# valida-xyz/valida

Measured on AMD Instinct MI355X. Metric: proofs/sec, 2^20-row Fibonacci trace, higher is better.
Workload: dtype u32; 1 GPU; C2: Fibonacci 2^20 cpu rows (mem 2^22), 14 chips, one proof per GPU; field=BabyBear / Ext5, mmcs=Keccak-256, fri_blowup=2, log_blowup=1, num_queries=40, pow_bits=8, parallelism=single GPU, proofs_in_flight_per_gpu=3, comm_stuck=False

## Files before the change

### bindings/rust/src/lib.rs

```rust
#![allow(non_camel_case_types, dead_code)]
use core::ffi::{c_char, c_int, c_void};

pub const VGPU_CBOR_CANONICAL_FIELDS: u32 = 1;
pub const VGPU_CBOR_PLAIN_DIGESTS: u32 = 2;
pub const VGPU_CBOR_IN_BARE_IS_MONTGOMERY: u32 = 1;
pub const VGPU_CBOR_SAW_FIELD_STRUCT: u32 = 1;
pub const VGPU_CBOR_SAW_FIELD_BARE: u32 = 2;
pub const VGPU_CBOR_SAW_DIGEST_STRUCT: u32 = 4;
pub const VGPU_CBOR_SAW_DIGEST_PLAIN: u32 = 8;
pub const VGPU_COMM_ID_BYTES: u32 = 128;
pub const VGPU_OK: i32 = 0;
pub const VGPU_ERR_INVALID_ARG: i32 = -1;
pub const VGPU_ERR_OOM: i32 = -2;
pub const VGPU_ERR_HIP: i32 = -3;
pub const VGPU_ERR_UNSUPPORTED: i32 = -4;
pub const VGPU_ERR_INTERNAL: i32 = -5;
pub const VGPU_ERR_FABRIC: i32 = -6;
pub const VGPU_HASH_KECCAK256: i32 = 0;
pub const VGPU_HASH_POSEIDON16: i32 = 1;
pub const VGPU_CPU_STORE32: i32 = 0;
pub const VGPU_CPU_LOAD32: i32 = 1;
pub const VGPU_CPU_JAL: i32 = 2;
pub const VGPU_CPU_JALV: i32 = 3;
pub const VGPU_CPU_BEQ: i32 = 4;
// ... 276 lines not shown
    pub alu2: [*const VgpuAluOp; 4],
    pub n_alu2: [u64; 4],
    pub output: *const VgpuOutOp,
    pub n_output: u64,
}

#[link(name = "vgpu")]
extern "C" {
    pub fn vgpu_last_error() -> *const c_char;
    pub fn vgpu_version() -> *const c_char;
    pub fn vgpu_air_new(name: *const c_char, width: u32, preprocessed_width: u32, out: *mut *mut VgpuAir) -> i32;
    pub fn vgpu_air_free(air: *mut VgpuAir);
    pub fn vgpu_air_constant(air: *mut VgpuAir, canonical: u32) -> u32;
    pub fn vgpu_air_variable(air: *mut VgpuAir, is_preprocessed: u32, column: u32, is_next: u32) -> u32;
    pub fn vgpu_air_is_first_row(air: *mut VgpuAir) -> u32;
    pub fn vgpu_air_is_last_row(air: *mut VgpuAir) -> u32;
    pub fn vgpu_air_is_transition(air: *mut VgpuAir) -> u32;
    pub fn vgpu_air_add(air: *mut VgpuAir, a: u32, b: u32) -> u32;
    pub fn vgpu_air_sub(air: *mut VgpuAir, a: u32, b: u32) -> u32;
    pub fn vgpu_air_mul(air: *mut VgpuAir, a: u32, b: u32) -> u32;
    pub fn vgpu_air_neg(air: *mut VgpuAir, a: u32) -> u32;
    pub fn vgpu_air_assert_zero(air: *mut VgpuAir, node: u32);
    pub fn vgpu_air_add_interaction(air: *mut VgpuAir, it: *const VgpuInteraction) -> i32;
    pub fn vgpu_machine_new(out: *mut *mut VgpuMachine) -> i32;
    pub fn vgpu_machine_push_air(m: *mut VgpuMachine, air: *const VgpuAir) -> i32;
    pub fn vgpu_machine_basic(out: *mut *mut VgpuMachine) -> i32;
    pub fn vgpu_machine_basic_via_ffi(out: *mut *mut VgpuMachine) -> i32;
    pub fn vgpu_machine_free(m: *mut VgpuMachine);
    pub fn vgpu_machine_num_chips(m: *const VgpuMachine) -> u32;
    pub fn vgpu_machine_chip_info(m: *const VgpuMachine, chip: u32, out: *mut u32) -> i32;
    pub fn vgpu_machine_interaction_words(m: *const VgpuMachine, chip: u32, out: *mut u32, cap: u64) -> i64;
    pub fn vgpu_machine_eval_constraints(m: *const VgpuMachine, chip: u32, main_local: *const u32, main_next: *const u32, prep_local: *const u32, prep_next: *const u32, is_first: u32, is_last: u32, is_transition: u32, out: *mut u32, cap: u32) -> i32;
    pub fn vgpu_challenger_new(poseidon_rc: *const u32, out: *mut *mut VgpuChallenger) -> i32;
    pub fn vgpu_challenger_free(ch: *mut VgpuChallenger);
    pub fn vgpu_challenger_observe(ch: *mut VgpuChallenger, values: *const u32, n: u64);
    pub fn vgpu_challenger_sample(ch: *mut VgpuChallenger, out: *mut u32, n: u64);
    pub fn vgpu_challenger_sample_bits(ch: *mut VgpuChallenger, bits: u32) -> u64;
    pub fn vgpu_challenger_grind(ch: *mut VgpuChallenger, bits: u32) -> u32;
    pub fn vgpu_poseidon16_permute(poseidon_rc: *const u32, state: *mut u32);
    pub fn vgpu_poseidon16_permute_sparse(poseidon_rc: *const u32, state: *mut u32) -> i32;
    pub fn vgpu_prover_create(cfg: *const VgpuConfig, machine: *const VgpuMachine, out: *mut *mut VgpuProver) -> i32;
    pub fn vgpu_prover_destroy(p: *mut VgpuProver);
    pub fn vgpu_prover_memory(p: *const VgpuProver, live_bytes: *mut u64, peak_bytes: *mut u64);
    pub fn vgpu_prover_trim(p: *mut VgpuProver) -> u64;
    pub fn vgpu_prover_memory_reset_peak(p: *mut VgpuProver);
    pub fn vgpu_prover_set_dense_lane(p: *mut VgpuProver, on: u32, min_nodes: u64);
    pub fn vgpu_prover_set_const_columns(p: *mut VgpuProver, on: u32);
    pub fn vgpu_prover_lane_stats(p: *const VgpuProver, entered: *mut u64, waited: *mut u64);
    pub fn vgpu_prover_set_profiling(p: *mut VgpuProver, on: u32);
    pub fn vgpu_prover_set_prep_cache(p: *mut VgpuProver, on: u32);
    pub fn vgpu_prover_set_profiling_filter(p: *mut VgpuProver, kernel_name: *const c_char);
    pub fn vgpu_prover_profile(p: *mut VgpuProver, out: *mut c_char, cap: u64) -> i64;
    pub fn vgpu_shader_clock_probe(device: i32, iters: u32, out: *mut u64) -> i32;
    pub fn vgpu_host_alloc(bytes: u64, out: *mut *mut c_void) -> i32;
    pub fn vgpu_host_free(ptr: *mut c_void);
    pub fn vgpu_trace_upload(p: *mut VgpuProver, data: *const u32, height: u64, width: u64, out: *mut *mut VgpuTrace) -> i32;
    pub fn vgpu_trace_free(t: *mut VgpuTrace);
    pub fn vgpu_commit_batches(p: *mut VgpuProver, mats: *const *const VgpuTrace, n_mats: u32, coset_shifts: *const u32, root: *mut u32, out: *mut *mut VgpuPdata) -> i32;
    pub fn vgpu_commit_batches_flagged(p: *mut VgpuProver, mats: *const *const VgpuTrace, n_mats: u32, root: *mut u32, out: *mut *mut VgpuPdata, varies_out: *mut u32) -> i32;
    pub fn vgpu_pdata_lde(p: *mut VgpuProver, pd: *const VgpuPdata, idx: u32, out: *mut u32, cap_words: u64) -> i32;
    pub fn vgpu_pdata_num_matrices(pd: *const VgpuPdata) -> u32;
    pub fn vgpu_pdata_lde_view(pd: *const VgpuPdata, idx: u32, out: *mut VgpuLdeView) -> i32;
    pub fn vgpu_pdata_free(pd: *mut VgpuPdata);
    pub fn vgpu_perm_trace(p: *mut VgpuProver, chip: u32, main: *const VgpuTrace, preprocessed_or_null: *const VgpuTrace, challenges: *const u32, out: *mut u32, cap_words: u64, cumulative_sum: *mut u32) -> i32;
    pub fn vgpu_perm_trace_device(p: *mut VgpuProver, chip: u32, main: *const VgpuTrace, preprocessed_or_null: *const VgpuTrace, challenges: *const u32, out: *mut *mut VgpuTrace, cumulative_sum: *mut u32) -> i32;
    pub fn vgpu_quotient(p: *mut VgpuProver, chip: u32, prep_pd: *const VgpuPdata, prep_idx: u32, main_pd: *const VgpuPdata, main_idx: u32, perm_pd: *const VgpuPdata, perm_idx: u32, perm_challenges: *const u32, alpha: *const u32, cumulative_sum: *const u32, out: *mut *mut VgpuTrace) -> i32;
    pub fn vgpu_open_multi_batches(p: *mut VgpuProver, rounds: *const *const VgpuPdata, n_rounds: u32, n_points: *const u32, points: *const u32, ch: *mut VgpuChallenger, out: *mut *mut VgpuOpening) -> i32;
    pub fn vgpu_opening_values_len(o: *const VgpuOpening) -> u64;
    pub fn vgpu_opening_values(o: *const VgpuOpening) -> *const u32;
    pub fn vgpu_opening_proof_len(o: *const VgpuOpening) -> u64;
    pub fn vgpu_opening_proof(o: *const VgpuOpening) -> *const u32;
    pub fn vgpu_opening_free(o: *mut VgpuOpening);
    pub fn vgpu_verify_multi_batches(cfg: *const VgpuConfig, commits: *const u32, n_rounds: u32, n_mats: *const u32, heights: *const u64, widths: *const u32, n_points: *const u32, points: *const u32, values: *const u32, n_value_words: u64, proof: *const u32, n_proof_words: u64, ch: *mut VgpuChallenger) -> i32;
    pub fn vgpu_verify(cfg: *const VgpuConfig, machine: *const VgpuMachine, preprocessed_commit: *const u32, proof_words: *const u32, n_words: u64) -> i32;
    pub fn vgpu_verifier_create(cfg: *const VgpuConfig, machine: *const VgpuMachine, out: *mut *mut VgpuVerifier) -> i32;
    pub fn vgpu_verifier_destroy(v: *mut VgpuVerifier);
    pub fn vgpu_verifier_set_chunk_words(v: *mut VgpuVerifier, chunk_words: u64) -> i32;
    pub fn vgpu_verify_batch(v: *mut VgpuVerifier, proofs: *const *const u32, n_words: *const u64, preprocessed_commits: *const u32, n_proofs: u32, status: *mut i32) -> i32;
    pub fn vgpu_verifier_message(v: *const VgpuVerifier, i: u32, out: *mut c_char, cap: u64) -> i64;
    pub fn vgpu_verifier_timing(v: *const VgpuVerifier, host_ms: *mut f64, device_ms: *mut f64);
    pub fn vgpu_host_commit_root(cfg: *const VgpuConfig, mats: *const *const u32, heights: *const u64, widths: *const u64, n_mats: u32, coset_shifts: *const u32, root: *mut u32) -> i32;
    pub fn vgpu_fri_fold(p: *mut VgpuProver, f: *const u32, n: u64, beta: *const u32, out: *mut u32) -> i32;
    pub fn vgpu_field_probe(p: *mut VgpuProver, op: u32, operands: *const u32, operand_words: u64, n_items: u64, results: *mut u32, result_words: u64) -> i32;
    pub fn vgpu_prover_set_pool_poison(p: *mut VgpuProver, mode: u32, word: u32) -> i32;
    pub fn vgpu_prover_pool_poison_stats(p: *const VgpuProver, out: *mut u64);
    pub fn vgpu_prover_pool_peek(p: *mut VgpuProver, bytes: u64, out: *mut u32, n_words: u64) -> i32;
    pub fn vgpu_verifier_set_poison(v: *mut VgpuVerifier, on: u32, word: u32) -> i32;
    pub fn vgpu_prove(p: *mut VgpuProver, main: *const *const VgpuTrace, n_main: u32, prep_chips: *const u32, prep: *const *const VgpuTrace, n_prep: u32, debug_flags: u32, out: *mut *mut VgpuProof) -> i32;
    pub fn vgpu_prove_async(p: *mut VgpuProver, main: *const *const VgpuTrace, n_main: u32, prep_chips: *const u32, prep: *const *const VgpuTrace, n_prep: u32, out: *mut *mut VgpuTicket) -> i32;
    pub fn vgpu_ticket_wait(t: *mut VgpuTicket, out: *mut *mut VgpuProof) -> i32;
    pub fn vgpu_proof_cbor(proof_words: *const u32, n_words: u64, flags: u32, out: *mut u8, cap_bytes: u64) -> i64;
    pub fn vgpu_proof_from_cbor(bytes: *const u8, n_bytes: u64, out: *mut u32, cap_words: u64) -> i64;
    pub fn vgpu_proof_from_cbor_ex(bytes: *const u8, n_bytes: u64, flags: u32, out: *mut u32, cap_words: u64, forms_seen: *mut u32) -> i64;
    pub fn vgpu_proof_len(pr: *const VgpuProof) -> u64;
    pub fn vgpu_proof_words(pr: *const VgpuProof) -> *const u32;
    pub fn vgpu_proof_phase_ms(pr: *const VgpuProof, out: *mut f64);
    pub fn vgpu_proof_transcript(pr: *const VgpuProof, out: *mut u32);
    pub fn vgpu_proof_debug_perm_trace(pr: *const VgpuProof, chip: u32, out: *mut u32, cap_words: u64) -> i64;
    pub fn vgpu_proof_debug_quotient(pr: *const VgpuProof, chip: u32, out: *mut u32, cap_words: u64) -> i64;
    pub fn vgpu_proof_free(pr: *mut VgpuProof);
    pub fn vgpu_bus_audit(p: *mut VgpuProver, main: *const *const VgpuTrace, n_main: u32, prep_chips: *const u32, prep: *const *const VgpuTrace, n_prep: u32, opts: *const VgpuBusAuditOpts, out: *mut *mut VgpuBusReport) -> i32;
    pub fn vgpu_bus_audit_host(machine: *const VgpuMachine, main: *const *const u32, heights: *const u64, widths: *const u64, n_main: u32, prep_chips: *const u32, prep: *const *const u32, prep_heights: *const u64, prep_widths: *const u64, n_prep: u32, opts: *const VgpuBusAuditOpts, out: *mut *mut VgpuBusReport) -> i32;
    pub fn vgpu_bus_report_len(r: *const VgpuBusReport) -> u64;
    pub fn vgpu_bus_report_words(r: *const VgpuBusReport) -> *const u32;
    pub fn vgpu_bus_report_timing(r: *const VgpuBusReport, out: *mut f64);
    pub fn vgpu_bus_report_free(r: *mut VgpuBusReport);
    pub fn vgpu_constraint_audit(p: *mut VgpuProver, main: *const *const VgpuTrace, n_main: u32, prep_chips: *const u32, prep: *const *const VgpuTrace, n_prep: u32, opts: *const VgpuConstraintAuditOpts, out: *mut *mut VgpuConstraintReport) -> i32;
    pub fn vgpu_constraint_audit_host(machine: *const VgpuMachine, main: *const *const u32, heights: *const u64, widths: *const u64, n_main: u32, prep_chips: *const u32, prep: *const *const u32, prep_heights: *const u64, prep_widths: *const u64, n_prep: u32, opts: *const VgpuConstraintAuditOpts, out: *mut *mut VgpuConstraintReport) -> i32;
    pub fn vgpu_constraint_report_len(r: *const VgpuConstraintReport) -> u64;
    pub fn vgpu_constraint_report_words(r: *const VgpuConstraintReport) -> *const u32;
    pub fn vgpu_constraint_report_timing(r: *const VgpuConstraintReport, out: *mut f64);
    pub fn vgpu_constraint_report_free(r: *mut VgpuConstraintReport);
    pub fn vgpu_mutation_audit(p: *mut VgpuProver, main: *const *const VgpuTrace, n_main: u32, prep_chips: *const u32, prep: *const *const VgpuTrace, n_prep: u32, opts: *const VgpuMutationAuditOpts, out: *mut *mut VgpuMutationReport) -> i32;
    pub fn vgpu_mutation_audit_host(machine: *const VgpuMachine, main: *const *const u32, heights: *const u64, widths: *const u64, n_main: u32, prep_chips: *const u32, prep: *const *const u32, prep_heights: *const u64, prep_widths: *const u64, n_prep: u32, opts: *const VgpuMutationAuditOpts, out: *mut *mut VgpuMutationReport) -> i32;
    pub fn vgpu_mutation_report_len(r: *const VgpuMutationReport) -> u64;
    pub fn vgpu_mutation_report_words(r: *const VgpuMutationReport) -> *const u32;
    pub fn vgpu_mutation_report_timing(r: *const VgpuMutationReport, out: *mut f64);
    pub fn vgpu_mutation_report_free(r: *mut VgpuMutationReport);
    pub fn vgpu_pair_audit(p: *mut VgpuProver, main: *const *const VgpuTrace, n_main: u32, prep_chips: *const u32, prep: *const *const VgpuTrace, n_prep: u32, opts: *const VgpuPairAuditOpts, out: *mut *mut VgpuPairReport) -> i32;
    pub fn vgpu_pair_audit_host(machine: *const VgpuMachine, main: *const *const u32, heights: *const u64, widths: *const u64, n_main: u32, prep_chips: *const u32, prep: *const *const u32, prep_heights: *const u64, prep_widths: *const u64, n_prep: u32, opts: *const VgpuPairAuditOpts, out: *mut *mut VgpuPairReport) -> i32;
    pub fn vgpu_pair_report_len(r: *const VgpuPairReport) -> u64;
    pub fn vgpu_pair_report_words(r: *const VgpuPairReport) -> *const u32;
    pub fn vgpu_pair_report_timing(r: *const VgpuPairReport, out: *mut f64);
    pub fn vgpu_pair_report_free(r: *mut VgpuPairReport);
    pub fn vgpu_rank_audit(p: *mut VgpuProver, main: *const *const VgpuTrace, n_main: u32, prep_chips: *const u32, prep: *const *const VgpuTrace, n_prep: u32, opts: *const VgpuRankAuditOpts, out: *mut *mut VgpuRankReport) -> i32;
    pub fn vgpu_rank_audit_host(machine: *const VgpuMachine, main: *const *const u32, heights: *const u64, widths: *const u64, n_main: u32, prep_chips: *const u32, prep: *const *const u32, prep_heights: *const u64, prep_widths: *const u64, n_prep: u32, opts: *const VgpuRankAuditOpts, out: *mut *mut VgpuRankReport) -> i32;
    pub fn vgpu_rank_report_len(r: *const VgpuRankReport) -> u64;
    pub fn vgpu_rank_report_words(r: *const VgpuRankReport) -> *const u32;
    pub fn vgpu_rank_report_timing(r: *const VgpuRankReport, out: *mut f64);
    pub fn vgpu_rank_report_free(r: *mut VgpuRankReport);
    pub fn vgpu_field_audit(p: *mut VgpuProver, main: *const *const VgpuTrace, n_main: u32, prep_chips: *const u32, prep: *const *const VgpuTrace, n_prep: u32, opts: *const VgpuRankAuditOpts, out: *mut *mut VgpuFieldReport) -> i32;
    pub fn vgpu_field_audit_host(machine: *const VgpuMachine, main: *const *const u32, heights: *const u64, widths: *const u64, n_main: u32, prep_chips: *const u32, prep: *const *const u32, prep_heights: *const u64, prep_widths: *const u64, n_prep: u32, opts: *const VgpuRankAuditOpts, out: *mut *mut VgpuFieldReport) -> i32;
    pub fn vgpu_field_report_len(r: *const VgpuFieldReport) -> u64;
    pub fn vgpu_field_report_words(r: *const VgpuFieldReport) -> *const u32;
    pub fn vgpu_field_report_timing(r: *const VgpuFieldReport, out: *mut f64);
    pub fn vgpu_field_report_free(r: *mut VgpuFieldReport);
    pub fn vgpu_link_audit(p: *mut VgpuProver, main: *const *const VgpuTrace, n_main: u32, prep_chips: *const u32, prep: *const *const VgpuTrace, n_prep: u32, opts: *const VgpuLinkAuditOpts, out: *mut *mut VgpuLinkReport) -> i32;
    pub fn vgpu_link_audit_host(machine: *const VgpuMachine, main: *const *const u32, heights: *const u64, widths: *const u64, n_main: u32, prep_chips: *const u32, prep: *const *const u32, prep_heights: *const u64, prep_widths: *const u64, n_prep: u32, opts: *const VgpuLinkAuditOpts, out: *mut *mut VgpuLinkReport) -> i32;
    pub fn vgpu_link_report_len(r: *const VgpuLinkReport) -> u64;
    pub fn vgpu_link_report_words(r: *const VgpuLinkReport) -> *const u32;
    pub fn vgpu_link_report_timing(r: *const VgpuLinkReport, out: *mut f64);
    pub fn vgpu_link_report_free(r: *mut VgpuLinkReport);
    pub fn vgpu_step_audit(p: *mut VgpuProver, main: *const *const VgpuTrace, n_main: u32, prep_chips: *const u32, prep: *const *const VgpuTrace, n_prep: u32, opts: *const VgpuStepAuditOpts, out: *mut *mut VgpuStepReport) -> i32;
    pub fn vgpu_step_audit_host(machine: *const VgpuMachine, main: *const *const u32, heights: *const u64, widths: *const u64, n_main: u32, prep_chips: *const u32, prep: *const *const u32, prep_heights: *const u64, prep_widths: *const u64, n_prep: u32, opts: *const VgpuStepAuditOpts, out: *mut *mut VgpuStepReport) -> i32;
    pub fn vgpu_step_report_len(r: *const VgpuStepReport) -> u64;
    pub fn vgpu_step_report_words(r: *const VgpuStepReport) -> *const u32;
    pub fn vgpu_step_report_timing(r: *const VgpuStepReport, out: *mut f64);
    pub fn vgpu_step_report_free(r: *mut VgpuStepReport);
    pub fn vgpu_invariant_audit(p: *mut VgpuProver, main: *const *const VgpuTrace, n_main: u32, prep_chips: *const u32, prep: *const *const VgpuTrace, n_prep: u32, opts: *const VgpuInvariantAuditOpts, out: *mut *mut VgpuInvariantReport) -> i32;
    pub fn vgpu_invariant_audit_host(machine: *const VgpuMachine, main: *const *const u32, heights: *const u64, widths: *const u64, n_main: u32, prep_chips: *const u32, prep: *const *const u32, prep_heights: *const u64, prep_widths: *const u64, n_prep: u32, opts: *const VgpuInvariantAuditOpts, out: *mut *mut VgpuInvariantReport) -> i32;
    pub fn vgpu_invariant_report_len(r: *const VgpuInvariantReport) -> u64;
    pub fn vgpu_invariant_report_words(r: *const VgpuInvariantReport) -> *const u32;
    pub fn vgpu_invariant_report_timing(r: *const VgpuInvariantReport, out: *mut f64);
    pub fn vgpu_invariant_report_free(r: *mut VgpuInvariantReport);
    pub fn vgpu_transition_audit(p: *mut VgpuProver, main: *const *const VgpuTrace, n_main: u32, prep_chips: *const u32, prep: *const *const VgpuTrace, n_prep: u32, opts: *const VgpuTransitionAuditOpts, out: *mut *mut VgpuTransitionReport) -> i32;
    pub fn vgpu_transition_audit_host(machine: *const VgpuMachine, main: *const *const u32, heights: *const u64, widths: *const u64, n_main: u32, prep_chips: *const u32, prep: *const *const u32, prep_heights: *const u64, prep_widths: *const u64, n_prep: u32, opts: *const VgpuTransitionAuditOpts, out: *mut *mut VgpuTransitionReport) -> i32;
    pub fn vgpu_transition_report_len(r: *const VgpuTransitionReport) -> u64;
    pub fn vgpu_transition_report_words(r: *const VgpuTransitionReport) -> *const u32;
    pub fn vgpu_transition_report_timing(r: *const VgpuTransitionReport, out: *mut f64);
    pub fn vgpu_transition_report_free(r: *mut VgpuTransitionReport);
    pub fn vgpu_product_audit(p: *mut VgpuProver, main: *const *const VgpuTrace, n_main: u32, prep_chips: *const u32, prep: *const *const VgpuTrace, n_prep: u32, opts: *const VgpuProductAuditOpts, out: *mut *mut VgpuProductReport) -> i32;
    pub fn vgpu_product_audit_host(machine: *const VgpuMachine, main: *const *const u32, heights: *const u64, widths: *const u64, n_main: u32, prep_chips: *const u32, prep: *const *const u32, prep_heights: *const u64, prep_widths: *const u64, n_prep: u32, opts: *const VgpuProductAuditOpts, out: *mut *mut VgpuProductReport) -> i32;
    pub fn vgpu_product_report_len(r: *const VgpuProductReport) -> u64;
    pub fn vgpu_product_report_words(r: *const VgpuProductReport) -> *const u32;
    pub fn vgpu_product_report_timing(r: *const VgpuProductReport, out: *mut f64);
    pub fn vgpu_product_report_free(r: *mut VgpuProductReport);
// ... 58 lines not shown
```

### include/vgpu.h

```cpp
#ifndef VGPU_H
#define VGPU_H
#include <stdint.h>
#ifdef __cplusplus
extern "C" {
#endif

enum {
    VGPU_OK = 0,
    VGPU_ERR_INVALID_ARG = -1,
    VGPU_ERR_OOM = -2,
    VGPU_ERR_HIP = -3,
    VGPU_ERR_UNSUPPORTED = -4,
    VGPU_ERR_INTERNAL = -5,
    VGPU_ERR_FABRIC = -6
};
enum {
    VGPU_HASH_KECCAK256 = 0,
    VGPU_HASH_POSEIDON16 = 1
};

const char* vgpu_last_error(void);
const char* vgpu_version(void);

typedef struct vgpu_config {
// ... 54 lines not shown
uint32_t vgpu_challenger_grind(vgpu_challenger_t* ch, uint32_t bits);
void vgpu_poseidon16_permute(const uint32_t poseidon_rc[480], uint32_t state[16]);
int32_t vgpu_poseidon16_permute_sparse(const uint32_t poseidon_rc[480], uint32_t state[16]);

typedef struct vgpu_prover vgpu_prover_t;
typedef struct vgpu_trace vgpu_trace_t;
typedef struct vgpu_pdata vgpu_pdata_t;
typedef struct vgpu_proof vgpu_proof_t;

int32_t vgpu_prover_create(const vgpu_config_t* cfg, const vgpu_machine_t* machine, vgpu_prover_t** out);
void vgpu_prover_destroy(vgpu_prover_t* p);
void vgpu_prover_memory(const vgpu_prover_t* p, uint64_t* live_bytes, uint64_t* peak_bytes);
uint64_t vgpu_prover_trim(vgpu_prover_t* p);
void vgpu_prover_memory_reset_peak(vgpu_prover_t* p);
void vgpu_prover_set_dense_lane(vgpu_prover_t* p, uint32_t on, uint64_t min_nodes);
void vgpu_prover_set_const_columns(vgpu_prover_t* p, uint32_t on);
void vgpu_prover_lane_stats(const vgpu_prover_t* p, uint64_t* entered, uint64_t* waited);

void vgpu_prover_set_profiling(vgpu_prover_t* p, uint32_t on);
void vgpu_prover_set_prep_cache(vgpu_prover_t* p, uint32_t on);
void vgpu_prover_set_profiling_filter(vgpu_prover_t* p, const char* kernel_name);
int64_t vgpu_prover_profile(vgpu_prover_t* p, char* out, uint64_t cap);
int32_t vgpu_shader_clock_probe(int32_t device, uint32_t iters, uint64_t out[2]);

int32_t vgpu_host_alloc(uint64_t bytes, void** out);
void vgpu_host_free(void* ptr);

int32_t vgpu_trace_upload(vgpu_prover_t* p, const uint32_t* data, uint64_t height, uint64_t width, vgpu_trace_t** out);
void vgpu_trace_free(vgpu_trace_t* t);

int32_t vgpu_commit_batches(vgpu_prover_t* p, const vgpu_trace_t* const* mats, uint32_t n_mats, const uint32_t* coset_shifts,
                            uint32_t root[8], vgpu_pdata_t** out);
int32_t vgpu_commit_batches_flagged(vgpu_prover_t* p, const vgpu_trace_t* const* mats, uint32_t n_mats, uint32_t root[8], vgpu_pdata_t** out,
                                    uint32_t* varies_out);
int32_t vgpu_pdata_lde(vgpu_prover_t* p, const vgpu_pdata_t* pd, uint32_t idx, uint32_t* out, uint64_t cap_words);
typedef struct vgpu_lde_view {
    const uint32_t* data;
    uint64_t height, width, stride;
    uint32_t log_blowup;
} vgpu_lde_view_t;
uint32_t vgpu_pdata_num_matrices(const vgpu_pdata_t* pd);
int32_t vgpu_pdata_lde_view(const vgpu_pdata_t* pd, uint32_t idx, vgpu_lde_view_t* out);
void vgpu_pdata_free(vgpu_pdata_t* pd);

int32_t vgpu_perm_trace(vgpu_prover_t* p, uint32_t chip, const vgpu_trace_t* main, const vgpu_trace_t* preprocessed_or_null,
                        const uint32_t challenges[15], uint32_t* out, uint64_t cap_words, uint32_t cumulative_sum[5]);

int32_t vgpu_perm_trace_device(vgpu_prover_t* p, uint32_t chip, const vgpu_trace_t* main, const vgpu_trace_t* preprocessed_or_null,
                               const uint32_t challenges[15], vgpu_trace_t** out, uint32_t cumulative_sum[5]);

int32_t vgpu_quotient(vgpu_prover_t* p, uint32_t chip, const vgpu_pdata_t* prep_pd, uint32_t prep_idx, const vgpu_pdata_t* main_pd, uint32_t main_idx,
                      const vgpu_pdata_t* perm_pd, uint32_t perm_idx, const uint32_t perm_challenges[15], const uint32_t alpha[5],
                      const uint32_t cumulative_sum[5], vgpu_trace_t** out);

typedef struct vgpu_opening vgpu_opening_t;
int32_t vgpu_open_multi_batches(vgpu_prover_t* p, const vgpu_pdata_t* const* rounds, uint32_t n_rounds, const uint32_t* n_points,
                                const uint32_t* points, vgpu_challenger_t* ch, vgpu_opening_t** out);
uint64_t vgpu_opening_values_len(const vgpu_opening_t* o);
const uint32_t* vgpu_opening_values(const vgpu_opening_t* o);
uint64_t vgpu_opening_proof_len(const vgpu_opening_t* o);
const uint32_t* vgpu_opening_proof(const vgpu_opening_t* o);
void vgpu_opening_free(vgpu_opening_t* o);

int32_t vgpu_verify_multi_batches(const vgpu_config_t* cfg, const uint32_t* commits, uint32_t n_rounds, const uint32_t* n_mats, const uint64_t* heights,
                                  const uint32_t* widths, const uint32_t* n_points, const uint32_t* points, const uint32_t* values, uint64_t n_value_words,
                                  const uint32_t* proof, uint64_t n_proof_words, vgpu_challenger_t* ch);

int32_t vgpu_verify(const vgpu_config_t* cfg, const vgpu_machine_t* machine, const uint32_t* preprocessed_commit, const uint32_t* proof_words,
                    uint64_t n_words);
typedef struct vgpu_verifier vgpu_verifier_t;
int32_t vgpu_verifier_create(const vgpu_config_t* cfg, const vgpu_machine_t* machine, vgpu_verifier_t** out);
void vgpu_verifier_destroy(vgpu_verifier_t* v);
int32_t vgpu_verifier_set_chunk_words(vgpu_verifier_t* v, uint64_t chunk_words);
int32_t vgpu_verify_batch(vgpu_verifier_t* v, const uint32_t* const* proofs, const uint64_t* n_words, const uint32_t* preprocessed_commits,
                          uint32_t n_proofs, int32_t* status);
int64_t vgpu_verifier_message(const vgpu_verifier_t* v, uint32_t i, char* out, uint64_t cap);
void vgpu_verifier_timing(const vgpu_verifier_t* v, double* host_ms, double* device_ms);
int32_t vgpu_host_commit_root(const vgpu_config_t* cfg, const uint32_t* const* mats, const uint64_t* heights, const uint64_t* widths, uint32_t n_mats,
                              const uint32_t* coset_shifts, uint32_t root[8]);

int32_t vgpu_fri_fold(vgpu_prover_t* p, const uint32_t* f, uint64_t n, const uint32_t beta[5], uint32_t* out);

int32_t vgpu_field_probe(vgpu_prover_t* p, uint32_t op, const uint32_t* operands, uint64_t operand_words, uint64_t n_items, uint32_t* results, uint64_t result_words);

int32_t vgpu_prover_set_pool_poison(vgpu_prover_t* p, uint32_t mode, uint32_t word);
void vgpu_prover_pool_poison_stats(const vgpu_prover_t* p, uint64_t out[4]);
int32_t vgpu_prover_pool_peek(vgpu_prover_t* p, uint64_t bytes, uint32_t* out, uint64_t n_words);
int32_t vgpu_verifier_set_poison(vgpu_verifier_t* v, uint32_t on, uint32_t word);

int32_t vgpu_prove(vgpu_prover_t* p, const vgpu_trace_t* const* main, uint32_t n_main, const uint32_t* prep_chips,
                   const vgpu_trace_t* const* prep, uint32_t n_prep, uint32_t debug_flags, vgpu_proof_t** out);
typedef struct vgpu_ticket vgpu_ticket_t;
int32_t vgpu_prove_async(vgpu_prover_t* p, const vgpu_trace_t* const* main, uint32_t n_main, const uint32_t* prep_chips,
                         const vgpu_trace_t* const* prep, uint32_t n_prep, vgpu_ticket_t** out);
int32_t vgpu_ticket_wait(vgpu_ticket_t* t, vgpu_proof_t** out);
#define VGPU_CBOR_CANONICAL_FIELDS 1u
#define VGPU_CBOR_PLAIN_DIGESTS 2u
int64_t vgpu_proof_cbor(const uint32_t* proof_words, uint64_t n_words, uint32_t flags, uint8_t* out, uint64_t cap_bytes);
int64_t vgpu_proof_from_cbor(const uint8_t* bytes, uint64_t n_bytes, uint32_t* out, uint64_t cap_words);
#define VGPU_CBOR_IN_BARE_IS_MONTGOMERY 1u
#define VGPU_CBOR_SAW_FIELD_STRUCT 1u
#define VGPU_CBOR_SAW_FIELD_BARE 2u
#define VGPU_CBOR_SAW_DIGEST_STRUCT 4u
#define VGPU_CBOR_SAW_DIGEST_PLAIN 8u
int64_t vgpu_proof_from_cbor_ex(const uint8_t* bytes, uint64_t n_bytes, uint32_t flags, uint32_t* out, uint64_t cap_words, uint32_t* forms_seen);
uint64_t vgpu_proof_len(const vgpu_proof_t* pr);
const uint32_t* vgpu_proof_words(const vgpu_proof_t* pr);
void vgpu_proof_phase_ms(const vgpu_proof_t* pr, double out[11]);
void vgpu_proof_transcript(const vgpu_proof_t* pr, uint32_t out[33]);
int64_t vgpu_proof_debug_perm_trace(const vgpu_proof_t* pr, uint32_t chip, uint32_t* out, uint64_t cap_words);
int64_t vgpu_proof_debug_quotient(const vgpu_proof_t* pr, uint32_t chip, uint32_t* out, uint64_t cap_words);
void vgpu_proof_free(vgpu_proof_t* pr);

typedef struct vgpu_bus_audit_opts { uint64_t max_tuples; uint32_t max_records_per_tuple; uint32_t hash_bits; } vgpu_bus_audit_opts_t;
typedef struct vgpu_bus_report vgpu_bus_report_t;
int32_t vgpu_bus_audit(vgpu_prover_t* p, const vgpu_trace_t* const* main, uint32_t n_main, const uint32_t* prep_chips, const vgpu_trace_t* const* prep,
                       uint32_t n_prep, const vgpu_bus_audit_opts_t* opts, vgpu_bus_report_t** out);
int32_t vgpu_bus_audit_host(const vgpu_machine_t* machine, const uint32_t* const* main, const uint64_t* heights, const uint64_t* widths, uint32_t n_main,
                            const uint32_t* prep_chips, const uint32_t* const* prep, const uint64_t* prep_heights, const uint64_t* prep_widths, uint32_t n_prep,
                            const vgpu_bus_audit_opts_t* opts, vgpu_bus_report_t** out);
uint64_t vgpu_bus_report_len(const vgpu_bus_report_t* r);
const uint32_t* vgpu_bus_report_words(const vgpu_bus_report_t* r);
void vgpu_bus_report_timing(const vgpu_bus_report_t* r, double out[2]);
void vgpu_bus_report_free(vgpu_bus_report_t* r);

typedef struct vgpu_constraint_audit_opts { uint64_t max_constraints; uint32_t max_rows_per_constraint; uint32_t reserved; } vgpu_constraint_audit_opts_t;
typedef struct vgpu_constraint_report vgpu_constraint_report_t;
int32_t vgpu_constraint_audit(vgpu_prover_t* p, const vgpu_trace_t* const* main, uint32_t n_main, const uint32_t* prep_chips, const vgpu_trace_t* const* prep,
                              uint32_t n_prep, const vgpu_constraint_audit_opts_t* opts, vgpu_constraint_report_t** out);
int32_t vgpu_constraint_audit_host(const vgpu_machine_t* machine, const uint32_t* const* main, const uint64_t* heights, const uint64_t* widths, uint32_t n_main,
                                   const uint32_t* prep_chips, const uint32_t* const* prep, const uint64_t* prep_heights, const uint64_t* prep_widths, uint32_t n_prep,
                                   const vgpu_constraint_audit_opts_t* opts, vgpu_constraint_report_t** out);
uint64_t vgpu_constraint_report_len(const vgpu_constraint_report_t* r);
const uint32_t* vgpu_constraint_report_words(const vgpu_constraint_report_t* r);
void vgpu_constraint_report_timing(const vgpu_constraint_report_t* r, double out[2]);
void vgpu_constraint_report_free(vgpu_constraint_report_t* r);

typedef struct vgpu_mutation_audit_opts {
    uint64_t max_entries;
    uint32_t max_rows_per_entry;
    uint32_t n_deltas;
    uint32_t deltas[4];
    uint32_t reserved[2];
} vgpu_mutation_audit_opts_t;
typedef struct vgpu_mutation_report vgpu_mutation_report_t;
int32_t vgpu_mutation_audit(vgpu_prover_t* p, const vgpu_trace_t* const* main, uint32_t n_main, const uint32_t* prep_chips, const vgpu_trace_t* const* prep,
                            uint32_t n_prep, const vgpu_mutation_audit_opts_t* opts, vgpu_mutation_report_t** out);
int32_t vgpu_mutation_audit_host(const vgpu_machine_t* machine, const uint32_t* const* main, const uint64_t* heights, const uint64_t* widths, uint32_t n_main,
                                 const uint32_t* prep_chips, const uint32_t* const* prep, const uint64_t* prep_heights, const uint64_t* prep_widths, uint32_t n_prep,
                                 const vgpu_mutation_audit_opts_t* opts, vgpu_mutation_report_t** out);
uint64_t vgpu_mutation_report_len(const vgpu_mutation_report_t* r);
const uint32_t* vgpu_mutation_report_words(const vgpu_mutation_report_t* r);
void vgpu_mutation_report_timing(const vgpu_mutation_report_t* r, double out[3]);
void vgpu_mutation_report_free(vgpu_mutation_report_t* r);

typedef struct vgpu_pair_audit_opts {
    uint64_t max_entries;
    uint32_t max_rows_per_entry;
    uint32_t n_deltas;
    uint32_t deltas[4];
    uint32_t chip_mask;
    uint32_t reserved;
} vgpu_pair_audit_opts_t;
typedef struct vgpu_pair_report vgpu_pair_report_t;
int32_t vgpu_pair_audit(vgpu_prover_t* p, const vgpu_trace_t* const* main, uint32_t n_main, const uint32_t* prep_chips, const vgpu_trace_t* const* prep,
                        uint32_t n_prep, const vgpu_pair_audit_opts_t* opts, vgpu_pair_report_t** out);
// ... 290 lines not shown
```

### valida_amd/__init__.py

```python
import ctypes
import os

import numpy as np

P = 2013265921
NUM_CHIPS = 14
CHIP_NAMES = ["cpu", "program", "mem", "add", "sub", "mul", "div", "shift", "lt", "com", "bitwise", "output", "range", "static_data"]

_HERE = os.path.dirname(os.path.abspath(__file__))
_LIB_PATH = os.environ.get("VGPU_LIB_PATH") or os.path.join(_HERE, "libvgpu.so")

c_u32p = ctypes.POINTER(ctypes.c_uint32)
c_u64p = ctypes.POINTER(ctypes.c_uint64)


HASH_KECCAK256, HASH_POSEIDON16 = 0, 1


class VgpuError(RuntimeError):
    def __init__(self, code, msg):
        super().__init__("vgpu error %d: %s" % (code, msg))
        self.code = code


# ... 241 lines not shown
        w = np.zeros(int(n), dtype=np.uint32)
        L.vgpu_machine_interaction_words(self._h, ctypes.c_uint32(chip), w.ctypes.data_as(c_u32p), ctypes.c_uint64(w.size))
        return decode_interaction_words(w)

    def eval_constraints(self, chip, main_local, main_next, prep_local=None, prep_next=None, is_first=0, is_last=0, is_transition=1):
        info = self.chip_info(chip)
        pl = np.zeros(max(1, info["preprocessed_width"]), dtype=np.uint32) if prep_local is None else prep_local
        pn = np.zeros(max(1, info["preprocessed_width"]), dtype=np.uint32) if prep_next is None else prep_next
        a, ap = _u32(main_local)
        b, bp = _u32(main_next)
        c, cp = _u32(pl)
        d, dp = _u32(pn)
        out = np.zeros(max(1, info["constraints"]), dtype=np.uint32)
        n = lib().vgpu_machine_eval_constraints(self._h, ctypes.c_uint32(chip), ap, bp, cp, dp, ctypes.c_uint32(is_first), ctypes.c_uint32(is_last),
                                                ctypes.c_uint32(is_transition), out.ctypes.data_as(c_u32p), ctypes.c_uint32(out.size))
        if n < 0:
            _check(n)
        return out[:n]

    def __del__(self):
        if getattr(self, "_h", None):
            try:
                lib().vgpu_machine_free(self._h)
            except TypeError:
                pass
            self._h = None


class Challenger:

    def __init__(self, rc):
        self._rc, rcp = _u32(rc)
        self._h = ctypes.c_void_p()
        _check(lib().vgpu_challenger_new(rcp, ctypes.byref(self._h)))

    def observe(self, values):
        v, vp = _u32(values)
        lib().vgpu_challenger_observe(self._h, vp, ctypes.c_uint64(v.size))

    def sample(self, n=1):
        out = np.zeros(n, dtype=np.uint32)
        lib().vgpu_challenger_sample(self._h, out.ctypes.data_as(c_u32p), ctypes.c_uint64(n))
        return out

    def sample_bits(self, bits):
        return int(lib().vgpu_challenger_sample_bits(self._h, ctypes.c_uint32(bits)))

    def grind(self, bits):
        return int(lib().vgpu_challenger_grind(self._h, ctypes.c_uint32(bits)))

    def __del__(self):
        if getattr(self, "_h", None):
            try:
                lib().vgpu_challenger_free(self._h)
            except TypeError:
                pass
            self._h = None


def poseidon16_permute(rc, state):
    r, rp = _u32(rc)
    s = np.array(state, dtype=np.uint32)
    lib().vgpu_poseidon16_permute(rp, s.ctypes.data_as(c_u32p))
    return s


FIELD_PROBE_OPS = {name: (code, iw, ow) for code, (name, iw, ow) in enumerate([
    ("reduce_once", 1, 1), ("sub_mod", 2, 1), ("add", 2, 1), ("sub", 2, 1), ("neg", 1, 1), ("mul", 2, 1), ("monty_reduce", 2, 1), ("monty_reduce_wide", 2, 1),
    ("from_canonical", 1, 1), ("canonical", 1, 1), ("inv", 1, 1), ("ext_mul", 10, 5), ("ext_square", 5, 5), ("ext_scale", 6, 5), ("ext_inv", 5, 5),
    ("bfly_dit_lb0", 18, 16), ("bfly_dit", 18, 16), ("bfly_dif_lb0", 18, 16), ("bfly_dif", 18, 16), ("monty_signed", 2, 1), ("sbox", 1, 1), ("sbox_plus", 2, 1),
    ("permute", 16, 16), ("permute_plain", 16, 16)])}


def field_probe(prover, op, operands):
    code, iw, ow = FIELD_PROBE_OPS[op]
    a = np.ascontiguousarray(operands, dtype=np.uint32)
    if a.ndim != 2 or a.shape[1] != iw or a.shape[0] == 0:
        raise ValueError("field_probe(%s): operands must be a non-empty (n_items, %d) array" % (op, iw))
    n = a.shape[0]
    src = np.ascontiguousarray(a.T)
    out = np.zeros((ow, n), dtype=np.uint32)
    _check(lib().vgpu_field_probe(prover._h, ctypes.c_uint32(code), src.ctypes.data_as(c_u32p), ctypes.c_uint64(src.size), ctypes.c_uint64(n),
                                  out.ctypes.data_as(c_u32p), ctypes.c_uint64(out.size)))
    return np.ascontiguousarray(out.T)


class _PinnedBlock:
    def __init__(self, nbytes):
        self.ptr = ctypes.c_void_p()
        _check(lib().vgpu_host_alloc(ctypes.c_uint64(max(1, nbytes)), ctypes.byref(self.ptr)))

    def __del__(self):
        if getattr(self, "ptr", None):
            try:
                lib().vgpu_host_free(self.ptr)
            except TypeError:
                pass
            self.ptr = None


def pinned_empty(shape, dtype=np.uint32):
    shape = (shape,) if isinstance(shape, int) else tuple(shape)
    dt = np.dtype(dtype)
    n = int(np.prod(shape)) if shape else 1
    blk = _PinnedBlock(n * dt.itemsize)
    buf = (ctypes.c_char * max(1, n * dt.itemsize)).from_address(blk.ptr.value)
    buf._vgpu_block = blk
    return np.frombuffer(buf, dtype=dt, count=n).reshape(shape)


def pinned_copy(a):
    out = pinned_empty(a.shape, a.dtype)
    out[...] = a
    return out


class DeviceOplog:
    def __init__(self, prover, handle, nbytes):
        self._prover, self._h, self.nbytes = prover, handle, nbytes

    def __del__(self):
        if getattr(self, "_h", None):
            try:
                lib().vgpu_oplog_free(self._h)
            except TypeError:
                pass
            self._h = None


class DeviceTrace:
    def __init__(self, prover, handle, shape):
        self._prover, self._h, self.shape = prover, handle, shape

    def download(self):
        out = np.zeros(self.shape, dtype=np.uint32)
        _check(lib().vgpu_trace_download(self._prover._h, self._h, out.ctypes.data_as(c_u32p), ctypes.c_uint64(out.size)))
        return out

    def __del__(self):
        if getattr(self, "_h", None):
            try:
                lib().vgpu_trace_free(self._h)
            except TypeError:
                pass
            self._h = None


class ProverData:

    def __init__(self, prover, handle, root, shapes):
        self._prover, self._h, self.root, self._shapes = prover, handle, root, shapes

    def lde(self, idx):
        h, w = self._shapes[idx]
        H = h << self._prover.log_blowup
        out = np.zeros((H, w), dtype=np.uint32)
        _check(lib().vgpu_pdata_lde(self._prover._h, self._h, ctypes.c_uint32(idx), out.ctypes.data_as(c_u32p), ctypes.c_uint64(out.size)))
        return out

    def lde_view(self, idx):

        class _View(ctypes.Structure):
            _fields_ = [("data", ctypes.c_void_p), ("height", ctypes.c_uint64), ("width", ctypes.c_uint64), ("stride", ctypes.c_uint64), ("log_blowup", ctypes.c_uint32)]

        v = _View()
        _check(lib().vgpu_pdata_lde_view(self._h, ctypes.c_uint32(idx), ctypes.byref(v)))
# ... 1908 lines not shown
```

### valida_amd/build.py

```python
import concurrent.futures
import os
import subprocess
import sys

ROOT = os.path.dirname(os.path.dirname(os.path.abspath(__file__)))
CSRC = os.path.join(ROOT, "valida_amd", "csrc")
BUILD = os.path.join(ROOT, "build")
LIB = os.path.join(ROOT, "valida_amd", "libvgpu.so")

SOURCES = [
    "kernels/ntt.hip",
    "kernels/layout.hip",
    "kernels/merkle.hip",
    "kernels/poseidon_mmcs.hip",
    "kernels/perm.hip",
    "kernels/quotient.hip",
    "kernels/open.hip",
    "kernels/tracegen.hip",
    "kernels/verify.hip",
    "kernels/bus_audit.hip",
    "kernels/constraint_audit.hip",
    "kernels/mutation_audit.hip",
    "kernels/coverage_audit.hip",
    "kernels/pair_audit.hip",
    "kernels/rank_audit.hip",
    "kernels/field_audit.hip",
    "kernels/link_audit.hip",
    "kernels/step_audit.hip",
    "kernels/invariant_audit.hip",
    "kernels/transition_audit.hip",
    "kernels/product_audit.hip",
    "kernels/domain_audit.hip",
    "kernels/memory_audit.hip",
    "kernels/program_audit.hip",
    "kernels/field_probe.hip",
    "host/prover.cpp",
    "host/prover_audits.cpp",
    "host/sharded_prover.cpp",
    "capi.cpp",
]
FLAGS = ["--offload-arch=gfx950", "-O3", "-std=c++17", "-fPIC", "-Wno-unused-result"]


def _newer_than(target, deps):
    if not os.path.exists(target):
        return False
    t = os.path.getmtime(target)
    return all(os.path.getmtime(d) <= t for d in deps)


def _all_headers():
    out = []
    for base, _, files in os.walk(CSRC):
        for f in files:
            if f.endswith((".hpp", ".h", ".inc")):
                out.append(os.path.join(base, f))
    out.append(os.path.join(ROOT, "include", "vgpu.h"))
    return out


LAST = {"compiled": [], "reused": [], "linked": False}
_FORCE = False


def _compile(src):
    obj = os.path.join(BUILD, src.replace("/", "_") + ".o")
    path = os.path.join(CSRC, src)
    if not _FORCE and _newer_than(obj, [path] + _all_headers()):
        LAST["reused"].append(src)
        return obj
    LAST["compiled"].append(src)
    cmd = ["hipcc"] + FLAGS + ["-x", "hip", "-c", path, "-o", obj]
    r = subprocess.run(cmd, capture_output=True, text=True)
    if r.returncode != 0:
        raise RuntimeError("hipcc failed for %s:\n%s" % (src, r.stderr))
    return obj


def build_vgpu(force=False):
    global _FORCE
    os.makedirs(BUILD, exist_ok=True)
    LAST["compiled"], LAST["reused"], LAST["linked"] = [], [], False
    srcs = [os.path.join(CSRC, s) for s in SOURCES]
    if not force and _newer_than(LIB, srcs + _all_headers()):
        LAST["reused"] = list(SOURCES)
        return LIB
    _FORCE = bool(force)
    with concurrent.futures.ThreadPoolExecutor(max_workers=8) as ex:
        objs = list(ex.map(_compile, SOURCES))
    tmp = os.path.join(BUILD, "libvgpu.%d.so" % os.getpid())
    cmd = ["hipcc", "--offload-arch=gfx950", "-shared", "-fPIC", "-o", tmp] + objs + ["-ldl"]
    r = subprocess.run(cmd, capture_output=True, text=True)
    if r.returncode != 0:
        if os.path.exists(tmp):
            os.unlink(tmp)
        raise RuntimeError("link failed:\n" + r.stderr)
    os.replace(tmp, LIB)
    LAST["linked"] = True
    return LIB


if __name__ == "__main__":
    print(build_vgpu("--force" in sys.argv))
```

### valida_amd/csrc/capi.cpp

```cpp
#include "../../include/vgpu.h"
#include <algorithm>
#include <cstring>
#include <future>
#include <map>
#include <mutex>
#include <memory>
#include <string>
#include "host/cbor.hpp"
#include "host/comm.hpp"
#include "host/sharded.hpp"
#include "host/sharded_prover.hpp"
#include "host/verifier.hpp"
#include "host/machine_verifier.hpp"
#include "host/verify_batch.hpp"
#include "host/poseidon_opt.hpp"
#include "host/prover.hpp"
#include "workload/basic_vm.hpp"
#include "workload/executable.hpp"

using namespace vhost;

static thread_local std::string g_err;
static int32_t fail(int32_t code, const std::string& msg) { g_err = msg; return code; }
#define VG_TRY(...)                                                         \
// ... 805 lines not shown
        std::vector<HostMatrixView> v;
        for (uint32_t i = 0; i < n_mats; i++) { if (!mats[i]) throw std::invalid_argument("null matrix"); v.push_back({mats[i], heights[i], widths[i]}); }
        Digest8 d = host_commit_root(v, coset_shifts, cfg->log_blowup, mmcs);
        memcpy(root, d.data(), 32);
    })
}
uint64_t vgpu_opening_values_len(const vgpu_opening_t* o) { return o->values.size(); }
const uint32_t* vgpu_opening_values(const vgpu_opening_t* o) { return o->values.data(); }
uint64_t vgpu_opening_proof_len(const vgpu_opening_t* o) { return o->proof.size(); }
const uint32_t* vgpu_opening_proof(const vgpu_opening_t* o) { return o->proof.data(); }
void vgpu_opening_free(vgpu_opening_t* o) { delete o; }

int32_t vgpu_perm_trace(vgpu_prover_t* p, uint32_t chip, const vgpu_trace_t* main, const vgpu_trace_t* prep, const uint32_t challenges[15], uint32_t* out,
                        uint64_t cap_words, uint32_t cumulative_sum[5]) {
    VG_TRY({
        if (!p || !main || !challenges || !out) throw std::invalid_argument("null argument");
        const MachineDesc& md = p->p->machine();
        if (chip >= md.airs.size()) throw std::invalid_argument("bad chip index");
        const AirDesc& air = md.airs[chip];
        if (main->t->width != air.width) throw std::invalid_argument("trace width mismatch");
        DeviceCtx& c = p->p->ctx();
        c.activate();
        DMat m = ingest(c, *main->t);
        DMat pm;
        if (prep) pm = ingest(c, *prep->t);
        Ext5 rnd[3];
        for (int i = 0; i < 3; i++) for (int k = 0; k < 5; k++) rnd[i].c[k] = Fp::from_canonical(challenges[5 * i + k]);
        uint32_t M = (uint32_t)air.interactions.size();
        std::vector<uint32_t> pool;
        size_t maxf = 0;
        for (auto& it : air.interactions) { put_ext(pool, (it.is_local() ? rnd[0] : rnd[1]).pow((uint64_t)it.bus_index + 1)); maxf = std::max(maxf, it.fields.size()); }
        Ext5 bp = Ext5::one();
        for (size_t j = 0; j < maxf; j++) { put_ext(pool, bp); bp *= rnd[2]; }
        pool.push_back(0);
        DBuf pool_dev(&c, pool), iw(&c, air.interaction_words), scratch(&c, (size_t)vk::perm_scratch_words(m.height));
        DMat perm(&c, m.height, 5 * (M + 1));
        if (cap_words < perm.height * perm.width) throw std::invalid_argument("output buffer too small");
        vk::launch_perm_trace(c.stream, m.view(), prep ? pm.view() : vk::DMatView{nullptr, 0, 0, 0}, iw.data, pool_dev.data, M, perm.view(), scratch.data);
        DBuf tmp(&c, (size_t)(perm.height * perm.width));
        vk::launch_export_rows(c.stream, perm.view(), 0, perm.height, tmp.data);
        c.check_launch("perm trace");
        c.download(out, tmp.data, perm.height * perm.width * 4);
        if (cumulative_sum) for (int k = 0; k < 5; k++) cumulative_sum[k] = out[(perm.height - 1) * perm.width + 5 * M + k];
    })
}

int32_t vgpu_fri_fold(vgpu_prover_t* p, const uint32_t* f, uint64_t n, const uint32_t beta[5], uint32_t* out) {
    VG_TRY({
        if (!p || !f || !beta || !out || n < 4 || (n & (n - 1))) throw std::invalid_argument("fri_fold: n must be a power of two >= 4");
        DeviceCtx& c = p->p->ctx();
        c.activate();
        uint64_t half = n / 2, q = half / 2;
        std::vector<uint32_t> in(5 * n);
        std::vector<uint32_t> bw(5);
        for (uint64_t i = 0; i < n; i++) for (int k = 0; k < 5; k++) in[((i & 1) * 5 + k) * half + (i >> 1)] = Fp::from_canonical(f[5 * i + k]).v;
        for (int k = 0; k < 5; k++) bw[k] = Fp::from_canonical(beta[k]).v;
        DBuf din(&c, in), dbeta(&c, bw), dout(&c, (size_t)(5 * half));
        vk::launch_fri_fold(c.stream, din.data, n, dbeta.data, nullptr, c.tables, dout.data);
        c.check_launch("fri fold");
        std::vector<uint32_t> o(5 * half);
        c.download(o.data(), dout.data, o.size() * 4);
        for (uint64_t i = 0; i < half; i++) for (int k = 0; k < 5; k++) out[5 * i + k] = Fp::raw(o[((i & 1) * 5 + k) * q + (i >> 1)]).canonical();
    })
}

int32_t vgpu_field_probe(vgpu_prover_t* p, uint32_t op, const uint32_t* operands, uint64_t operand_words, uint64_t n_items, uint32_t* results, uint64_t result_words) {
    VG_TRY({
        int iw = 0, ow = 0;
        if (!p || !operands || !results) throw std::invalid_argument("null argument");
        if (!vk::field_probe_shape(op, &iw, &ow)) throw std::invalid_argument("field probe: unknown op");
        if (n_items == 0 || n_items > (1ull << 24)) throw std::invalid_argument("field probe: 1 .. 2^24 items");
        if (operand_words != n_items * (uint64_t)iw || result_words != n_items * (uint64_t)ow) throw std::invalid_argument("field probe: buffer sizes do not match the op's shape");
        vk::field_probe_check_twiddle_range(op, operands, n_items);
        DeviceCtx& c = p->p->ctx();
        c.activate();
        DBuf din(&c, (size_t)operand_words), dout(&c, (size_t)result_words);
        c.upload(din.data, operands, operand_words * 4);
        vk::launch_field_probe(c.stream, op, din.data, n_items, c.tables, c.poseidon_tab, c.poseidon_sparse, dout.data);
        c.check_launch("field probe");
        c.download(results, dout.data, result_words * 4);
    })
}

int32_t vgpu_prover_set_pool_poison(vgpu_prover_t* p, uint32_t mode, uint32_t word) {
    VG_TRY({
        if (!p) throw std::invalid_argument("null argument");
        if (mode > 3) throw std::invalid_argument("pool poison: mode is bit 0 (on alloc) | bit 1 (on release)");
        DeviceCtx& c = p->p->ctx();
        std::unique_lock<std::mutex> owner(c.prove_mu, std::try_to_lock);
        if (!owner.owns_lock() || c.async_pending.load() > 0) throw std::invalid_argument("pool poison: a proof or an audit is running on this context");
        std::lock_guard<std::mutex> lk(c.pool_mu);
        c.poison_mode = mode;
        c.poison_word = word;
    })
}
void vgpu_prover_pool_poison_stats(const vgpu_prover_t* p, uint64_t out[4]) {
    if (!p || !out) return;
    DeviceCtx& c = const_cast<vgpu_prover_t*>(p)->p->ctx();
    std::lock_guard<std::mutex> lk(c.pool_mu);
    for (int i = 0; i < 4; i++) out[i] = c.poison_stats[i];
}
int32_t vgpu_prover_pool_peek(vgpu_prover_t* p, uint64_t bytes, uint32_t* out, uint64_t n_words) {
    VG_TRY({
        if (!p || !out) throw std::invalid_argument("null argument");
        if (!bytes || n_words > bytes / 4) throw std::invalid_argument("pool peek: bytes >= 1 and 4 * n_words <= bytes");
        DeviceCtx& c = p->p->ctx();
        c.activate();
        const size_t rounded = ((size_t)bytes + 255) & ~(size_t)255;
        DBuf b(&c, (size_t)((bytes + 3) / 4));
        std::vector<uint32_t> w(n_words + 1);
        if (n_words) c.download(w.data(), b.data, n_words * 4);
        c.download(w.data() + n_words, b.data + rounded / 4 - 1, 4);
        memcpy(out, w.data(), w.size() * 4);
    })
}

static void check_trace(const vgpu_prover_t* p, const vgpu_trace_t* t, std::vector<std::shared_ptr<Prover>>* foreign = nullptr) {
    if (!t || !t->t) throw std::invalid_argument("null trace");
    if (t->owner == p->p) return;
    if (!foreign || t->owner->ctx().device != p->p->ctx().device) throw std::invalid_argument("trace belongs to another prover context");
    if (std::find(foreign->begin(), foreign->end(), t->owner) == foreign->end()) foreign->push_back(t->owner);
}
static void drain(const std::vector<std::shared_ptr<Prover>>& ctxs) {
    for (auto& q : ctxs) { q->ctx().activate(); q->ctx().sync(); }
}

int32_t vgpu_prove(vgpu_prover_t* p, const vgpu_trace_t* const* main, uint32_t n_main, const uint32_t* prep_chips, const vgpu_trace_t* const* prep,
                   uint32_t n_prep, uint32_t debug_flags, vgpu_proof_t** out) {
    VG_TRY({
        if (!p || !main || !out || (n_prep && (!prep || !prep_chips))) throw std::invalid_argument("null argument");
        std::vector<const DeviceTrace*> m;
        std::vector<std::shared_ptr<Prover>> foreign;
        for (uint32_t i = 0; i < n_main; i++) { check_trace(p, main[i], &foreign); m.push_back(main[i]->t.get()); }
        std::vector<std::pair<int, const DeviceTrace*>> pr;
        for (uint32_t i = 0; i < n_prep; i++) { check_trace(p, prep[i], &foreign); pr.push_back({(int)prep_chips[i], prep[i]->t.get()}); }
        drain(foreign);
        auto proof = std::make_unique<vgpu_proof>();
        proof->dbg.keep_matrices = (debug_flags & 1) != 0;
        proof->dbg.check_constraints = (debug_flags & 2) != 0;
        proof->words = p->p->prove(m, pr, &proof->tm, &proof->dbg);
        *out = proof.release();
    })
}

extern "C++" {
template <class Report> static auto report_evaluations(const Report& rep, int) -> decltype(rep.evaluations) { return rep.evaluations; }
template <class Report> static double report_evaluations(const Report&, long) { return 0; }
template <class Handle, class Report>
static Handle* audit_report_handle(const Report& rep) {
    auto h = std::make_unique<Handle>();
    h->words = rep.words(); h->device_ms = rep.device_ms; h->host_ms = rep.host_ms; h->evaluations = report_evaluations(rep, 0);
    return h.release();
}
template <class Handle, class Audit>
static int32_t audit_on_device(vgpu_prover_t* p, const vgpu_trace_t* const* main, uint32_t n_main, const uint32_t* prep_chips, const vgpu_trace_t* const* prep, uint32_t n_prep, Handle** out,
                        Audit&& audit) {
    VG_TRY({
        if (!p || !out || (n_main && !main) || (n_prep && (!prep || !prep_chips))) throw std::invalid_argument("null argument");
        std::vector<const DeviceTrace*> m;
        std::vector<std::shared_ptr<Prover>> foreign;
        for (uint32_t i = 0; i < n_main; i++) { check_trace(p, main[i], &foreign); m.push_back(main[i]->t.get()); }
        std::vector<std::pair<int, const DeviceTrace*>> pr;
        for (uint32_t i = 0; i < n_prep; i++) { check_trace(p, prep[i], &foreign); pr.push_back({(int)prep_chips[i], prep[i]->t.get()}); }
        drain(foreign);
        *out = audit_report_handle<Handle>(audit(m, pr));
    })
// ... 861 lines not shown
```

### valida_amd/csrc/field.hpp

```cpp
#pragma once
#include <cstdint>

#if defined(__HIPCC__)
#include <hip/hip_runtime.h>
#define VG_HD __host__ __device__ __forceinline__
#else
#define VG_HD inline
#endif

namespace vg {

constexpr uint32_t P = 0x78000001u;
constexpr uint32_t P_INV_NEG = 0x77ffffffu;
constexpr uint32_t R_MOD_P = 268435454u;
constexpr uint32_t R2_MOD_P = 1172168163u;
constexpr uint32_t GENERATOR = 31;
constexpr uint32_t TWO_ADIC_ROOT_27 = 0x1a427a41u;

#ifndef VG_MULHI_NOP
#define VG_MULHI_NOP 0
#endif
VG_HD uint32_t mul_lo_pinv(uint32_t lo) {
#if defined(__HIP_DEVICE_COMPILE__) && VG_MULHI_NOP == 2
    uint32_t o;
    asm("v_mul_lo_u32 %0, %1, %2\n\ts_nop 0" : "=v"(o) : "v"(lo), "v"(0x88000001u));
    return o;
#else
    return lo * 0x88000001u;
#endif
}
VG_HD uint32_t mul_hi_u32(uint32_t a, uint32_t b) {
#if defined(__HIP_DEVICE_COMPILE__) && VG_MULHI_NOP
    uint32_t o;
    asm("v_mul_hi_u32 %0, %1, %2\n\ts_nop 0" : "=v"(o) : "v"(a), "v"(b));
    return o;
#elif defined(__HIP_DEVICE_COMPILE__)
    return __umulhi(a, b);
#else
    return (uint32_t)(((uint64_t)a * b) >> 32);
#endif
}

#ifndef VG_CARRY_REDUCE
#define VG_CARRY_REDUCE 1
#endif
#if defined(__HIP_DEVICE_COMPILE__) && VG_CARRY_REDUCE == 2
VG_HD uint32_t reduce_once(uint32_t s) {
    uint32_t t, r;
    asm("v_subrev_co_u32_e32 %0, vcc, %3, %2\n\tv_cndmask_b32_e32 %1, %0, %2, vcc" : "=&v"(t), "=v"(r) : "v"(s), "v"(P) : "vcc");
    return r;
}
VG_HD uint32_t sub_mod(uint32_t a, uint32_t b) {
    uint32_t d, t, r;
    asm("v_sub_co_u32_e32 %0, vcc, %3, %4\n\tv_add_u32_e32 %1, %5, %0\n\tv_cndmask_b32_e32 %2, %0, %1, vcc" : "=&v"(d), "=&v"(t), "=v"(r) : "v"(a), "v"(b), "v"(P) : "vcc");
    return r;
}
#elif defined(__HIP_DEVICE_COMPILE__) && VG_CARRY_REDUCE
VG_HD uint32_t reduce_once(uint32_t s) {
    uint32_t t, r;
    unsigned long long borrow;
    asm("v_subrev_co_u32_e64 %0, %1, %4, %3\n\tv_cndmask_b32_e64 %2, %0, %3, %1" : "=&v"(t), "=&s"(borrow), "=v"(r) : "v"(s), "v"(P));
    return r;
}
VG_HD uint32_t sub_mod(uint32_t a, uint32_t b) {
    uint32_t d, t, r;
    unsigned long long borrow;
    asm("v_sub_co_u32_e64 %0, %1, %4, %5\n\tv_add_u32_e32 %2, %6, %0\n\tv_cndmask_b32_e64 %3, %0, %2, %1" : "=&v"(d), "=&s"(borrow), "=&v"(t), "=v"(r) : "v"(a), "v"(b), "v"(P));
    return r;
}
#else
VG_HD uint32_t reduce_once(uint32_t s) { uint32_t t = s - P; return s < t ? s : t; }
VG_HD uint32_t sub_mod(uint32_t a, uint32_t b) { uint32_t d = a - b, t = d + P; return d < t ? d : t; }
#endif

#ifndef VG_MONTY_ADD
#define VG_MONTY_ADD 0
#endif
VG_HD uint32_t monty_reduce(uint64_t t) {
#if VG_MONTY_ADD == 1
    const uint32_t m = (uint32_t)t * P_INV_NEG;
    return reduce_once((uint32_t)((t + (uint64_t)m * P) >> 32));
#else
    uint32_t lo = (uint32_t)t, hi = (uint32_t)(t >> 32);
    uint32_t m = mul_lo_pinv(lo);
    uint32_t u = mul_hi_u32(m, P);
    return sub_mod(hi, u);
#endif
}

VG_HD uint32_t monty_reduce_wide(uint64_t t) {
    uint32_t lo = (uint32_t)t, hi = reduce_once((uint32_t)(t >> 32));
    uint32_t m = mul_lo_pinv(lo);
    uint32_t u = mul_hi_u32(m, P);
    return sub_mod(hi, u);
}

struct Fp {
    uint32_t v;
    VG_HD static Fp raw(uint32_t m) { Fp r; r.v = m; return r; }
    VG_HD static Fp zero() { return raw(0); }
    VG_HD static Fp one() { return raw(R_MOD_P); }
    VG_HD static Fp from_canonical(uint32_t x) { return raw(monty_reduce((uint64_t)x * R2_MOD_P)); }
    VG_HD uint32_t canonical() const { return monty_reduce((uint64_t)v); }
    VG_HD bool is_zero() const { return v == 0; }
    VG_HD bool operator==(const Fp& o) const { return v == o.v; }
    VG_HD bool operator!=(const Fp& o) const { return v != o.v; }
    VG_HD Fp operator+(const Fp& o) const { return raw(reduce_once(v + o.v)); }
    VG_HD Fp operator-(const Fp& o) const { return raw(sub_mod(v, o.v)); }
    VG_HD Fp operator-() const { return raw(v ? P - v : 0); }
#if VG_MONTY_ADD == 2 && defined(__HIP_DEVICE_COMPILE__)
    VG_HD Fp operator*(const Fp& o) const {
        uint32_t lo, hi;
        asm("v_mul_lo_u32 %0, %2, %3\n\tv_mul_hi_u32 %1, %2, %3" : "=&v"(lo), "=v"(hi) : "v"(v), "v"(o.v));
        return raw(sub_mod(hi, mul_hi_u32(lo * 0x88000001u, P)));
    }
#else
    VG_HD Fp operator*(const Fp& o) const { return raw(monty_reduce((uint64_t)v * o.v)); }
#endif
    VG_HD Fp& operator+=(const Fp& o) { *this = *this + o; return *this; }
    VG_HD Fp& operator-=(const Fp& o) { *this = *this - o; return *this; }
    VG_HD Fp& operator*=(const Fp& o) { *this = *this * o; return *this; }
    VG_HD Fp square() const { return *this * *this; }
    VG_HD Fp pow(uint64_t e) const {
        Fp r = one(), b = *this;
        while (e) { if (e & 1) r *= b; b *= b; e >>= 1; }
        return r;
    }
    VG_HD Fp exp_power_of_2(unsigned k) const { Fp r = *this; for (unsigned i = 0; i < k; i++) r *= r; return r; }
    VG_HD Fp inv() const {
        const Fp x = *this;
        const Fp x3 = x.square() * x, x7 = x3.square() * x;
        const Fp a6 = x7.exp_power_of_2(3) * x7;
        const Fp a12 = a6.exp_power_of_2(6) * a6;
        const Fp a24 = a12.exp_power_of_2(12) * a12;
        const Fp t = a24.exp_power_of_2(3) * x7;
        const Fp w = t * x, w2 = w.square(), w4 = w2.square(), w8 = w4.square();
        return t * (w8 * w4 * w2);
    }
    VG_HD Fp halve() const { return raw((v & 1) ? (uint32_t)(((uint64_t)v + P) >> 1) : v >> 1); }
};

VG_HD Fp two_adic_generator(unsigned bits) {
    return Fp::from_canonical(TWO_ADIC_ROOT_27).exp_power_of_2(27 - bits);
}

struct Ext5 {
    Fp c[5];
    VG_HD static Ext5 zero() { Ext5 r; for (int i = 0; i < 5; i++) r.c[i] = Fp::zero(); return r; }
    VG_HD static Ext5 one() { Ext5 r = zero(); r.c[0] = Fp::one(); return r; }
    VG_HD static Ext5 from_base(Fp b) { Ext5 r = zero(); r.c[0] = b; return r; }
    VG_HD bool is_zero() const { return (c[0].v | c[1].v | c[2].v | c[3].v | c[4].v) == 0; }
    VG_HD bool operator==(const Ext5& o) const { for (int i = 0; i < 5; i++) if (c[i].v != o.c[i].v) return false; return true; }
    VG_HD bool operator!=(const Ext5& o) const { return !(*this == o); }
    VG_HD Ext5 operator+(const Ext5& o) const { Ext5 r; for (int i = 0; i < 5; i++) r.c[i] = c[i] + o.c[i]; return r; }
    VG_HD Ext5 operator-(const Ext5& o) const { Ext5 r; for (int i = 0; i < 5; i++) r.c[i] = c[i] - o.c[i]; return r; }
    VG_HD Ext5 operator-() const { Ext5 r; for (int i = 0; i < 5; i++) r.c[i] = -c[i]; return r; }
    VG_HD Ext5 operator*(const Fp& s) const { Ext5 r; for (int i = 0; i < 5; i++) r.c[i] = c[i] * s; return r; }
    VG_HD Ext5 operator+(const Fp& s) const { Ext5 r = *this; r.c[0] += s; return r; }
    VG_HD Ext5 operator-(const Fp& s) const { Ext5 r = *this; r.c[0] -= s; return r; }
    VG_HD Ext5 operator*(const Ext5& o) const {
        Fp d[5];
#pragma unroll
        for (int j = 0; j < 5; j++) d[j] = o.c[j] + o.c[j];
        Ext5 r;
#pragma unroll
        for (int k = 0; k < 5; k++) {
            uint32_t bb[5];
#pragma unroll
            for (int i = 0; i < 5; i++) bb[i] = i <= k ? o.c[k - i].v : d[k + 5 - i].v;
            uint64_t t0123 = (uint64_t)c[0].v * bb[0] + (uint64_t)c[1].v * bb[1] + (uint64_t)c[2].v * bb[2] + (uint64_t)c[3].v * bb[3];
            uint64_t t4 = (uint64_t)c[4].v * bb[4];
            r.c[k] = Fp::raw(monty_reduce_wide(t0123)) + Fp::raw(monty_reduce(t4));
        }
        return r;
    }
    VG_HD Ext5& operator+=(const Ext5& o) { *this = *this + o; return *this; }
    VG_HD Ext5& operator-=(const Ext5& o) { *this = *this - o; return *this; }
    VG_HD Ext5& operator*=(const Ext5& o) { *this = *this * o; return *this; }
    VG_HD Ext5 square() const { return *this * *this; }
    VG_HD Ext5 pow(uint64_t e) const {
        Ext5 r = one(), b = *this;
        while (e) { if (e & 1) r *= b; b *= b; e >>= 1; }
        return r;
    }
    VG_HD Ext5 exp_power_of_2(unsigned k) const { Ext5 r = *this; for (unsigned i = 0; i < k; i++) r *= r; return r; }
    template <int K> VG_HD Ext5 frobenius_k() const {
        constexpr uint32_t Z[5] = {0, 1079828539u, 847078768u, 1597816133u, 233372948u};
        Ext5 r;
        r.c[0] = c[0];
        r.c[1] = c[1] * Fp::raw(Z[(1 * K) % 5]);
        r.c[2] = c[2] * Fp::raw(Z[(2 * K) % 5]);
        r.c[3] = c[3] * Fp::raw(Z[(3 * K) % 5]);
        r.c[4] = c[4] * Fp::raw(Z[(4 * K) % 5]);
        return r;
    }
    VG_HD Ext5 frobenius() const { return frobenius_k<1>(); }
    VG_HD Ext5 inv() const {
        Ext5 f1 = frobenius_k<1>(), f2 = frobenius_k<2>(), f3 = frobenius_k<3>(), f4 = frobenius_k<4>();
        Ext5 prod = (f1 * f2) * (f3 * f4);
        Fp hi = c[1] * prod.c[4] + c[2] * prod.c[3] + c[3] * prod.c[2] + c[4] * prod.c[1];
        Fp norm = c[0] * prod.c[0] + hi + hi;
        return prod * norm.inv();
    }
};

VG_HD uint32_t reverse_bits_len(uint32_t x, unsigned bits) {
#if defined(__HIP_DEVICE_COMPILE__)
    return bits ? (__brev(x) >> (32 - bits)) : 0;
#else
    uint32_t r = 0;
    for (unsigned i = 0; i < bits; i++) r |= ((x >> i) & 1u) << (bits - 1 - i);
    return r;
#endif
}

inline unsigned log2_strict_u64(uint64_t n) { unsigned k = 0; while ((1ull << k) < n) k++; return k; }

}
```

### valida_amd/csrc/kernels/launch.hpp

```cpp
#pragma once
#include <vector>
#include "device_common.hpp"
#include "profiler.hpp"
#include "../air/symbolic.hpp"
#include "verify_args.hpp"

namespace vk {

struct QuotientArgs {
    DMatView main_lde, perm_lde, prep_lde;
    int log_n;
    const vair::Instr* prog;
    uint32_t n_instrs, n_regs, n_air_asserts;
    const uint32_t* iw;
    const uint32_t* consts;
    uint32_t K;
    uint32_t coset_shift, coset_shift_inv;
    int lqd;
    uint32_t zh_inv[8];
    uint32_t zh[8];
    uint32_t g_inv;
    DMatView out;
    int out_natural;
    static constexpr int INTERPRET = -2;
    int native_chip;
    const uint32_t* main_nx;
    const uint32_t* perm_nx;
    const uint32_t* prep_nx;
    uint32_t next_step_p1;
    QuotientArgs normalised() const {
        QuotientArgs b = *this;
        if (!b.main_nx) b.main_nx = b.main_lde.data;
        if (!b.perm_nx) b.perm_nx = b.perm_lde.data;
        if (!b.prep_nx) b.prep_nx = b.prep_lde.data;
        if (!b.next_step_p1) b.next_step_p1 = 1u + (1u << (b.lqd > 0 ? b.lqd : 1));
        return b;
    }
};

constexpr uint32_t INTERP_LDS_MIN_THREADS = 64;
constexpr uint32_t INTERP_LDS_BYTES_PAIR = 148 * 1024, INTERP_LDS_BYTES_GENERAL = 160 * 1024;
constexpr uint32_t INTERP_LDS_MAX_REGS_PAIR = INTERP_LDS_BYTES_PAIR / (4 * INTERP_LDS_MIN_THREADS);
constexpr uint32_t INTERP_LDS_MAX_REGS_GENERAL = INTERP_LDS_BYTES_GENERAL / (4 * INTERP_LDS_MIN_THREADS);
constexpr uint32_t interp_lds_max_regs(unsigned lqd) { return lqd == 1 ? INTERP_LDS_MAX_REGS_PAIR : INTERP_LDS_MAX_REGS_GENERAL; }
inline unsigned interp_lds_threads(uint32_t n_regs) {
    unsigned threads = 256;
    while (threads > INTERP_LDS_MIN_THREADS && (size_t)n_regs * threads * 4 > 64 * 1024) threads >>= 1;
    return threads;
}

void launch_ingest(hipStream_t st, const uint32_t* src_dev, DMatView dst, bool bitrev, uint32_t* varies = nullptr);
constexpr uint64_t INGEST_FLAGS_MAX_WIDTH = 512;
void launch_bitrev_rows(hipStream_t st, DMatView src, DMatView dst);
void launch_clock_probe(hipStream_t st, uint64_t* out3, uint32_t iters);
void launch_interleave_blocks(hipStream_t st, const uint32_t* src, uint32_t* dst, uint64_t rows, uint32_t log_wq, uint64_t n_cols);
void launch_export_rows(hipStream_t st, DMatView src, uint64_t row0, uint64_t nrows, uint32_t* dst_dev);
enum FieldProbeOp {
    FP_REDUCE_ONCE = 0, FP_SUB_MOD, FP_ADD, FP_SUB, FP_NEG, FP_MUL, FP_MONTY_REDUCE, FP_MONTY_REDUCE_WIDE, FP_FROM_CANONICAL, FP_CANONICAL, FP_INV,
    FP_EXT_MUL, FP_EXT_SQUARE, FP_EXT_SCALE, FP_EXT_INV, FP_BFLY_DIT_LB0, FP_BFLY_DIT, FP_BFLY_DIF_LB0, FP_BFLY_DIF, FP_MONTY_SIGNED, FP_SBOX, FP_SBOX_PLUS,
    FP_PERMUTE, FP_PERMUTE_PLAIN, FIELD_PROBE_OPS
};
bool field_probe_shape(uint32_t op, int* in_words, int* out_words);
void field_probe_check_twiddle_range(uint32_t op, const uint32_t* in_host, uint64_t n);
void launch_field_probe(hipStream_t st, uint32_t op, const uint32_t* in_dev, uint64_t n, const DeviceTables& tb, const uint32_t* pos_dev, bool sparse, uint32_t* out_dev);
void launch_intt(hipStream_t st, DMatView m, const DeviceTables& tb);
void launch_coset_ntt(hipStream_t st, DMatView coeffs, DMatView dst, uint64_t dst_row0, Fp shift, const DeviceTables& tb);
void launch_lde_natural(hipStream_t st, DMatView nat, DMatView lde, int log_blowup, const DeviceTables& tb, const LdeTables& lt, DMatView s1, DMatView s2,
                        const uint32_t* colmap = nullptr);
constexpr uint32_t COLMAP_LIVE_COUNT = 0, COLMAP_CONST_COUNT = 1, COLMAP_LIVE = 2;
inline size_t lde_colmap_words(uint64_t width) { return 2 + 2 * (size_t)width; }
void launch_lde_colmap(hipStream_t st, const uint32_t* varies, uint64_t width, uint32_t* colmap);
void launch_verify_chunk(hipStream_t st, const VerifyChunkArgs& a);
void launch_keccak_leaves(hipStream_t st, const uint32_t* const* cols_dev, int n_elems, uint64_t n_rows, uint32_t* digests);
void launch_keccak_leaves_strided(hipStream_t st, const uint32_t* base, uint64_t stride, int n_elems, uint64_t n_rows, uint32_t* digests);
void launch_keccak_compress(hipStream_t st, const uint32_t* prev, const uint32_t* const* cols_dev, int n_elems, uint64_t n_out, uint32_t* next);
void launch_keccak_bottom_q(hipStream_t st, const uint32_t* jobs_dev, uint32_t n_jobs, const uint32_t* indices_dev, uint32_t* dst);
void launch_poseidon_bottom_q(hipStream_t st, const uint32_t* pos_dev, bool sparse, const uint32_t* jobs_dev, uint32_t n_jobs, const uint32_t* indices_dev, uint32_t* dst);
constexpr int KECCAK_TOP_MAX_LEVELS = 11;
struct KeccakTopArgs {
    const uint32_t* prev;
    uint64_t first_len;
    int levels;
    uint32_t* out[KECCAK_TOP_MAX_LEVELS];
    const uint32_t* const* cols[KECCAK_TOP_MAX_LEVELS];
    int n_elems[KECCAK_TOP_MAX_LEVELS];
    const uint32_t* leaf_base = nullptr;
    uint64_t leaf_stride = 0;
    int leaf_elems = 0;
    uint64_t leaf_rows = 0;
    uint64_t block_len = 0;
    const uint32_t* ch_pos = nullptr;
    uint32_t* ch_state = nullptr;
    uint32_t* ch_beta5 = nullptr;
    uint32_t* ch_commit8 = nullptr;
};
void launch_keccak_top(hipStream_t st, const KeccakTopArgs& a);
constexpr uint64_t KECCAK_LEVELS_BLOCK_LEN = 64;
void launch_keccak_levels(hipStream_t st, const KeccakTopArgs& a);
bool keccak_levels_fused(uint64_t len);
bool keccak_levels_take_leaves(uint64_t n_rows);
bool keccak_top_takes_leaves(uint64_t n_rows);
void launch_poseidon_leaves(hipStream_t st, const uint32_t* pos_dev, bool sparse, const uint32_t* const* cols_dev, int n_elems, uint64_t n_rows, uint32_t* digests);
void launch_poseidon_leaves_strided(hipStream_t st, const uint32_t* pos_dev, bool sparse, const uint32_t* base, uint64_t stride, int n_elems, uint64_t n_rows, uint32_t* digests);
void launch_poseidon_compress(hipStream_t st, const uint32_t* pos_dev, bool sparse, const uint32_t* prev, const uint32_t* const* cols_dev, int n_elems, uint64_t n_out, uint32_t* next);
bool poseidon_levels_take(uint64_t parents);
int poseidon_levels_group(uint64_t parents);
void launch_poseidon_levels(hipStream_t st, const uint32_t* pos_dev, bool sparse, const KeccakTopArgs& a);
void launch_poseidon_top(hipStream_t st, const uint32_t* pos_dev, bool sparse, const KeccakTopArgs& a);
uint64_t perm_scratch_words(uint64_t n);
void launch_add_ext_const(hipStream_t st, uint32_t* data, uint64_t stride, uint64_t n, const uint32_t* off5_dev);
void launch_perm_trace(hipStream_t st, DMatView main, DMatView prep, const uint32_t* iw_dev, const uint32_t* chal_dev, uint32_t M, DMatView perm,
                       uint32_t* scratch, int native_chip = -2);
void launch_quotient(hipStream_t st, const QuotientArgs& a, const DeviceTables& tb);
void launch_check_constraints(hipStream_t st, const QuotientArgs& a, unsigned long long* first_bad_dev);
struct TgCpuOp { uint32_t pc, fp, opcode; int32_t operands[5]; uint32_t kind, has_imm, imm, mem_first; };
struct TgMemOp { uint32_t clk, addr, value, is_write; };
struct TgAluOp { uint32_t opcode, a, b, c; };
struct TgOutOp { uint32_t clk, byte; };
enum { TG_CPU_STORE32 = 0, TG_CPU_LOAD32, TG_CPU_JAL, TG_CPU_JALV, TG_CPU_BEQ, TG_CPU_BNE, TG_CPU_IMM32, TG_CPU_BUS, TG_CPU_BUS_LEFT_IMM, TG_CPU_STOP,
       TG_CPU_LOADFP, TG_CPU_LOAD_U8, TG_CPU_LOAD_S8, TG_CPU_STORE_U8, TG_CPU_READ_ADVICE };
void launch_tracegen_cpu(hipStream_t st, const TgCpuOp* ops, uint64_t n, const TgMemOp* mem, uint64_t n_mem, DMatView t);
size_t tracegen_mem_sort_scratch_bytes(uint64_t n);
hipError_t launch_tracegen_mem(hipStream_t st, const TgMemOp* mem, uint64_t n, const uint32_t* static_cells, uint64_t n_static, uint32_t* keys2, uint32_t* idx2,
                               void* sort_tmp, size_t sort_tmp_bytes, DMatView t);
void launch_tracegen_alu(hipStream_t st, int chip, const TgAluOp* ops, uint64_t n, DMatView t);
void launch_tracegen_idle(hipStream_t st, int mode, const uint32_t* static_cells, uint64_t n_static, DMatView t);
hipError_t launch_tracegen_range(hipStream_t st, const TgCpuOp* ops, uint64_t n, const TgMemOp* mem, uint64_t n_mem, uint32_t* counts, DMatView t);
void launch_tracegen_alu2(hipStream_t st, int chip, const TgAluOp* ops, uint64_t n, DMatView t);
void launch_tracegen_output(hipStream_t st, const TgOutOp* vals, const uint32_t* row0, uint64_t n, uint64_t n_rows, DMatView t);
hipError_t launch_tracegen_program(hipStream_t st, const TgCpuOp* ops, uint64_t n, uint64_t padded_n, uint32_t rom_len, uint32_t* counts, DMatView t);
size_t bus_audit_sort_scratch_words(uint64_t n);
size_t bus_audit_scan_scratch_words(uint64_t n);
void launch_ba_records(hipStream_t st, const uint32_t* desc, uint32_t chip, uint64_t height, uint32_t width, uint32_t M, uint32_t hash_bits, unsigned long long* keys, uint32_t* ids,
                       uint32_t* cnt, uint32_t* live_out);
void launch_ba_iota(hipStream_t st, uint32_t* ids, uint64_t n);
void launch_ba_rekey(hipStream_t st, const uint32_t* desc, uint32_t chunk, const uint32_t* ids, const uint32_t* cnt, unsigned long long* keys, uint64_t n);
int launch_ba_sort(hipStream_t st, unsigned long long* keys2, uint32_t* vals2, uint64_t n, uint32_t* counts, const int* shifts, int n_shifts, int half);
void launch_ba_groups(hipStream_t st, const uint32_t* desc, const unsigned long long* keys, const uint32_t* ids, uint64_t n, bool exact, uint32_t* gid, uint32_t* head_pos,
                      uint32_t* scan_tmp, uint32_t* counters);
void launch_ba_reduce(hipStream_t st, const uint32_t* desc, const uint32_t* ids, const uint32_t* cnt, const uint32_t* gid, const uint32_t* head_pos, uint64_t n, bool check,
                      unsigned long long* sums, uint32_t* nrec, uint32_t* counters);
void launch_ba_select(hipStream_t st, const uint32_t* desc, const uint32_t* ids, const uint32_t* head_pos, const unsigned long long* sums, uint64_t n_groups_max, bool collect,
                      uint32_t cap, unsigned long long* ukeys, uint32_t* uvals, uint32_t* counters);
void launch_ba_report(hipStream_t st, const uint32_t* desc, const uint32_t* ids, const uint32_t* cnt, const uint32_t* head_pos, const unsigned long long* sums, const uint32_t* nrec,
                      const uint32_t* uvals, uint32_t n_rep, uint32_t R, uint32_t* out);
constexpr uint32_t CA_MAX_CONSTRAINTS = 96, CA_MASK_WORDS = 3;
constexpr int CA_INTERPRET = -2;
// ... 275 lines not shown
```

### valida_amd/csrc/kernels/open.hip

```cpp
#include <cstdlib>
#include <stdexcept>
#include <type_traits>
#include <vector>
#include <string>
#include "launch.hpp"
#include "poseidon_perm.hpp"
#include "challenger_dev.hpp"

namespace vk {

constexpr int BARY_ROWS = 4;
__device__ __forceinline__ void bary_weights_block(uint64_t block, uint64_t n, const uint32_t* __restrict__ mg, uint32_t shift, const DeviceTables& tb, uint32_t* __restrict__ w,
                                                   uint32_t* __restrict__ img) {
    const uint64_t j0 = (block * blockDim.x + threadIdx.x) * BARY_ROWS;
    if (j0 >= n) return;
    const uint32_t* g = mg + 5;
    Fp r[BARY_ROWS], mx[BARY_ROWS], pre[BARY_ROWS];
    Ext5 gx[BARY_ROWS];
    Fp run = Fp::one();
#pragma unroll
    for (int q = 0; q < BARY_ROWS; q++) {
        const bool live = j0 + q < n;
        r[q] = live ? domain_point(tb, (uint32_t)(j0 + q)) : Fp::one();
        const Fp x = Fp::raw(shift) * r[q], x2 = x * x, x3 = x2 * x, x4 = x2 * x2, x5 = x4 * x;
// ... 194 lines not shown
                const uint32_t d0 = __builtin_amdgcn_ubfe(v[q].x, 7 * a, 7), d1 = __builtin_amdgcn_ubfe(v[q].y, 7 * a, 7);
                const uint32_t d2 = __builtin_amdgcn_ubfe(v[q].z, 7 * a, 7), d3 = __builtin_amdgcn_ubfe(v[q].w, 7 * a, 7);
                B[a][q] = (int)(d0 | (d1 << 8) | (d2 << 16) | (d3 << 24));
            }
#pragma unroll
        for (int a = 0; a < 5; a++)
#pragma unroll
            for (int b = 0; b < 5; b++) acc[a + b] = __builtin_amdgcn_mfma_i32_16x16x64_i8(A[a], B[b], acc[a + b], 0, 0, 0);
#pragma unroll
        for (int a = 0; a < 5; a++) A[a] = An[a];
#pragma unroll
        for (int q = 0; q < 4; q++) v[q] = vn[q];
    }
    Fp pw[9];
    pw[0] = Fp::one();
    const Fp step = Fp::from_canonical(128);
#pragma unroll
    for (int s = 1; s < 9; s++) pw[s] = pw[s - 1] * step;
    const uint64_t n_out = C * PK;
#pragma unroll
    for (int r = 0; r < 4; r++) {
        const int pk = 4 * g + r;
        if (pk < PK && col_live) {
            Fp y = Fp::zero();
#pragma unroll
            for (int s = 0; s < 9; s++) y += Fp::from_canonical((uint32_t)acc[s][r]) * pw[s];
            partial[chunk * n_out + c * PK + pk] = vg::monty_reduce((uint64_t)vg::monty_reduce((uint64_t)y.v));
        }
    }
}

__global__ void __launch_bounds__(64) k_col_dot_finish(const uint32_t* __restrict__ partial, uint64_t n_blocks, uint64_t width, int NP, const uint32_t* __restrict__ scale5 ,
                                 uint32_t* __restrict__ out) {
    const uint64_t idx = blockIdx.x;
    const uint64_t c = idx / NP;
    const int p = (int)(idx % NP);
    const uint64_t n_out = width * NP * 5;
    Ext5 acc = Ext5::zero();
    for (uint64_t b = threadIdx.x; b < n_blocks; b += 64) acc += ext_from_words(partial + b * n_out + (c * NP + p) * 5);
#pragma unroll
    for (int k = 0; k < 5; k++) acc.c[k] = wave_sum(acc.c[k]);
    if (threadIdx.x == 0) {
        acc = acc * ext_from_words(scale5 + 5 * p);
        for (int k = 0; k < 5; k++) out[idx * 5 + k] = acc.c[k].canonical();
    }
}

struct DotFinishJob { uint32_t first_block, np; const uint32_t* partial; uint64_t n_blocks, width; const uint32_t* scale5; uint32_t* out; };
__global__ void __launch_bounds__(64) k_col_dot_finish_batch(const DotFinishJob* __restrict__ jobs, uint32_t n_jobs) {
    uint32_t lo = 0, hi = n_jobs - 1;
    while (lo < hi) { const uint32_t mid = (lo + hi + 1) >> 1; if (jobs[mid].first_block <= blockIdx.x) lo = mid; else hi = mid - 1; }
    const DotFinishJob j = jobs[lo];
    const uint64_t idx = blockIdx.x - j.first_block;
    const uint64_t c = idx / j.np;
    const int p = (int)(idx % j.np);
    const uint64_t n_out = j.width * j.np * 5;
    Ext5 acc = Ext5::zero();
    for (uint64_t b = threadIdx.x; b < j.n_blocks; b += 64) acc += ext_from_words(j.partial + b * n_out + (c * j.np + p) * 5);
#pragma unroll
    for (int k = 0; k < 5; k++) acc.c[k] = wave_sum(acc.c[k]);
    if (threadIdx.x == 0) {
        acc = acc * ext_from_words(j.scale5 + 5 * p);
        for (int k = 0; k < 5; k++) j.out[idx * 5 + k] = acc.c[k].canonical();
    }
}

constexpr int MAX_OPEN_POINTS = MAX_OPEN_POINTS_PER_LAUNCH;

__global__ void __launch_bounds__(256) k_reduce_openings(const uint32_t* __restrict__ desc, uint64_t L, uint32_t shift, DeviceTables tb, uint32_t* __restrict__ out, int accumulate) {
    uint64_t j = (uint64_t)blockIdx.x * blockDim.x + threadIdx.x;
    if (j >= L) return;
    const uint32_t n_mats = desc[0], n_points = desc[1], max_w = desc[2];
    const uint32_t* mg = desc + 3;
    const uint32_t* apow = mg + 25 * n_points;
    const uint32_t* md = apow + 5 * max_w;
    Ext5 S[MAX_OPEN_POINTS];
#pragma unroll
    for (int p = 0; p < MAX_OPEN_POINTS; p++) S[p] = Ext5::zero();
    for (uint32_t mi = 0; mi < n_mats; mi++) {
        const uint32_t* colp = reinterpret_cast<const uint32_t*>(((uint64_t)md[1] << 32) | md[0]);
        const uint64_t stride = ((uint64_t)md[3] << 32) | md[2];
        const uint32_t width = md[4], npts = md[5];
        md += 6;
        Ext5 rr = Ext5::zero();
        uint32_t c = 0;
        for (; c + 16 <= width; c += 16) {
            uint32_t v[16];
#pragma unroll
            for (int u = 0; u < 16; u++) v[u] = colp[(uint64_t)(c + u) * stride + j];
#pragma unroll
            for (int g = 0; g < 16; g += 4) {
                const uint32_t* a0 = apow + 5 * (c + g);
#pragma unroll
                for (int k = 0; k < 5; k++) {
                    uint64_t t = (uint64_t)a0[k] * v[g] + (uint64_t)a0[5 + k] * v[g + 1] + (uint64_t)a0[10 + k] * v[g + 2] + (uint64_t)a0[15 + k] * v[g + 3];
                    rr.c[k] += Fp::raw(vg::monty_reduce_wide(t));
                }
            }
        }
        for (; c + 4 <= width; c += 4) {
            const uint32_t v0 = colp[(uint64_t)c * stride + j], v1 = colp[(uint64_t)(c + 1) * stride + j];
            const uint32_t v2 = colp[(uint64_t)(c + 2) * stride + j], v3 = colp[(uint64_t)(c + 3) * stride + j];
            const uint32_t* a0 = apow + 5 * c;
#pragma unroll
            for (int k = 0; k < 5; k++) {
                uint64_t t = (uint64_t)a0[k] * v0 + (uint64_t)a0[5 + k] * v1 + (uint64_t)a0[10 + k] * v2 + (uint64_t)a0[15 + k] * v3;
                rr.c[k] += Fp::raw(vg::monty_reduce_wide(t));
            }
        }
        for (; c < width; c++) rr += ext_from_words(apow + 5 * c) * Fp::raw(colp[(uint64_t)c * stride + j]);
        for (uint32_t q = 0; q < npts; q++, md += 11) {
            Ext5 t = ext_from_words(md + 1) * (ext_from_words(md + 6) - rr);
            const uint32_t slot = md[0];
#pragma unroll
            for (int p = 0; p < MAX_OPEN_POINTS; p++) if ((uint32_t)p == slot) S[p] += t;
        }
    }
    const Fp x = Fp::raw(shift) * domain_point(tb, (uint32_t)j);
    const Fp x2 = x * x, x3 = x2 * x, x4 = x2 * x2, x5 = x4 * x;
    Ext5 gx[MAX_OPEN_POINTS];
    Fp mx[MAX_OPEN_POINTS], pre[MAX_OPEN_POINTS];
    Fp run = Fp::one();
#pragma unroll
    for (int p = 0; p < MAX_OPEN_POINTS; p++)
        if ((uint32_t)p < n_points) {
            const uint32_t* q = mg + 25 * p;
            const uint64_t tm = (uint64_t)q[1] * x.v + (uint64_t)q[2] * x2.v + (uint64_t)q[3] * x3.v + (uint64_t)q[4] * x4.v;
            mx[p] = Fp::raw(vg::monty_reduce_wide(tm)) + Fp::raw(q[0]) + x5;
            const uint32_t* g = q + 5;
#pragma unroll
            for (int k = 0; k < 5; k++) {
                const uint64_t tg = (uint64_t)g[5 + k] * x.v + (uint64_t)g[10 + k] * x2.v + (uint64_t)g[15 + k] * x3.v;
                gx[p].c[k] = Fp::raw(vg::monty_reduce_wide(tg)) + Fp::raw(g[k]);
            }
            gx[p].c[0] += x4;
            pre[p] = run;
            run = run * mx[p];
        }
    Fp inv_run = run.inv();
    Ext5 ro = Ext5::zero();
#pragma unroll
    for (int p = MAX_OPEN_POINTS - 1; p >= 0; p--)
        if ((uint32_t)p < n_points) { ro -= (S[p] * gx[p]) * (inv_run * pre[p]); inv_run = inv_run * mx[p]; }
    const uint64_t half = L >> 1;
    if (accumulate) ro += load_ext(out + (j & 1) * 5 * half, half, j >> 1);
    store_ext(out + (j & 1) * 5 * half, half, j >> 1, ro);
}

template <int R> struct RowVec;
template <> struct RowVec<2> { using T = uint2; static __device__ __forceinline__ void get(const T& v, uint32_t (&e)[2]) { e[0] = v.x; e[1] = v.y; } };
template <> struct RowVec<4> { using T = uint4; static __device__ __forceinline__ void get(const T& v, uint32_t (&e)[4]) { e[0] = v.x; e[1] = v.y; e[2] = v.z; e[3] = v.w; } };
template <int NP, int R>
__global__ void __launch_bounds__(256) k_reduce_openings_rows(const uint32_t* __restrict__ desc, uint64_t L, uint32_t shift, DeviceTables tb, uint32_t* __restrict__ out, int accumulate) {
    using V = typename RowVec<R>::T;
    const uint64_t j0 = ((uint64_t)blockIdx.x * blockDim.x + threadIdx.x) * R;
    if (j0 >= L) return;
    const uint32_t n_mats = desc[0], n_points = desc[1], max_w = desc[2];
    const uint32_t* mg = desc + 3;
    const uint32_t* apow = mg + 25 * n_points;
    const uint32_t* md = apow + 5 * max_w;
    Ext5 S[NP][R];
#pragma unroll
    for (int p = 0; p < NP; p++)
#pragma unroll
        for (int r = 0; r < R; r++) S[p][r] = Ext5::zero();
    for (uint32_t mi = 0; mi < n_mats; mi++) {
        const uint32_t* colp = reinterpret_cast<const uint32_t*>(((uint64_t)md[1] << 32) | md[0]) + j0;
        const uint64_t stride = ((uint64_t)md[3] << 32) | md[2];
        const uint32_t width = md[4], npts = md[5];
        md += 6;
        Ext5 rr[R];
#pragma unroll
        for (int r = 0; r < R; r++) rr[r] = Ext5::zero();
        auto four_cols = [&](const V& v0, const V& v1, const V& v2, const V& v3, const uint32_t* a0) {
            uint32_t e0[R], e1[R], e2[R], e3[R];
            RowVec<R>::get(v0, e0); RowVec<R>::get(v1, e1); RowVec<R>::get(v2, e2); RowVec<R>::get(v3, e3);
#pragma unroll
            for (int r = 0; r < R; r++)
#pragma unroll
                for (int k = 0; k < 5; k++) {
                    const uint64_t t = (uint64_t)a0[k] * e0[r] + (uint64_t)a0[5 + k] * e1[r] + (uint64_t)a0[10 + k] * e2[r] + (uint64_t)a0[15 + k] * e3[r];
                    rr[r].c[k] += Fp::raw(vg::monty_reduce_wide(t));
                }
        };
        uint32_t c = 0;
        for (; c + 8 <= width; c += 8) {
            V v[8];
#pragma unroll
            for (int u = 0; u < 8; u++) v[u] = *reinterpret_cast<const V*>(colp + (uint64_t)(c + u) * stride);
            four_cols(v[0], v[1], v[2], v[3], apow + 5 * c);
            four_cols(v[4], v[5], v[6], v[7], apow + 5 * (c + 4));
        }
        for (; c + 4 <= width; c += 4) {
            V v[4];
#pragma unroll
            for (int u = 0; u < 4; u++) v[u] = *reinterpret_cast<const V*>(colp + (uint64_t)(c + u) * stride);
            four_cols(v[0], v[1], v[2], v[3], apow + 5 * c);
        }
        for (; c < width; c++) {
            uint32_t e[R];
            RowVec<R>::get(*reinterpret_cast<const V*>(colp + (uint64_t)c * stride), e);
            const Ext5 a = ext_from_words(apow + 5 * c);
#pragma unroll
            for (int r = 0; r < R; r++) rr[r] += a * Fp::raw(e[r]);
        }
        for (uint32_t q = 0; q < npts; q++, md += 11) {
            const Ext5 coef = ext_from_words(md + 1), Y = ext_from_words(md + 6);
            const uint32_t slot = md[0];
#pragma unroll
            for (int r = 0; r < R; r++) {
                const Ext5 t = coef * (Y - rr[r]);
#pragma unroll
                for (int p = 0; p < NP; p++) if ((uint32_t)p == slot) S[p][r] += t;
            }
        }
    }
    const Fp x = Fp::raw(shift) * domain_point(tb, (uint32_t)j0), im = domain_point(tb, 2u);
    const Fp x2 = x * x, x3 = x2 * x, x4 = x2 * x2, x5 = x4 * x;
    Fp pw[R][5];
    pw[0][0] = x; pw[0][1] = x2; pw[0][2] = x3; pw[0][3] = x4; pw[0][4] = x5;
    pw[1][0] = -x; pw[1][1] = x2; pw[1][2] = -x3; pw[1][3] = x4; pw[1][4] = -x5;
    if constexpr (R == 4) {
        const Fp ix = im * x, ix3 = im * x3, ix5 = im * x5;
        pw[2][0] = ix; pw[2][1] = -x2; pw[2][2] = -ix3; pw[2][3] = x4; pw[2][4] = ix5;
        pw[3][0] = -ix; pw[3][1] = -x2; pw[3][2] = ix3; pw[3][3] = x4; pw[3][4] = -ix5;
    }
    Fp mx[NP][R], pre[NP][R];
    Fp run = Fp::one();
#pragma unroll
    for (int p = 0; p < NP; p++)
        if ((uint32_t)p < n_points) {
            const uint32_t* q = mg + 25 * p;
#pragma unroll
            for (int r = 0; r < R; r++) {
                const uint64_t tm = (uint64_t)q[1] * pw[r][0].v + (uint64_t)q[2] * pw[r][1].v + (uint64_t)q[3] * pw[r][2].v + (uint64_t)q[4] * pw[r][3].v;
                mx[p][r] = Fp::raw(vg::monty_reduce_wide(tm)) + Fp::raw(q[0]) + pw[r][4];
                pre[p][r] = run;
                run = run * mx[p][r];
            }
        }
    Fp inv_run = run.inv();
    Ext5 ro[R];
#pragma unroll
    for (int r = 0; r < R; r++) ro[r] = Ext5::zero();
    auto point_step = [&](auto pc) {
        constexpr int p = decltype(pc)::value;
        if ((uint32_t)p < n_points) {
            const uint32_t* g = mg + 25 * p + 5;
#pragma unroll
            for (int r = R - 1; r >= 0; r--) {
                Ext5 gx;
#pragma unroll
                for (int k = 0; k < 5; k++) {
                    const uint64_t tg = (uint64_t)g[5 + k] * pw[r][0].v + (uint64_t)g[10 + k] * pw[r][1].v + (uint64_t)g[15 + k] * pw[r][2].v;
                    gx.c[k] = Fp::raw(vg::monty_reduce_wide(tg)) + Fp::raw(g[k]);
                }
                gx.c[0] += pw[r][3];
                ro[r] -= (S[p][r] * gx) * (inv_run * pre[p][r]);
                inv_run = inv_run * mx[p][r];
            }
        }
    };
    if constexpr (NP > 3) point_step(std::integral_constant<int, 3>{});
    if constexpr (NP > 2) point_step(std::integral_constant<int, 2>{});
    if constexpr (NP > 1) point_step(std::integral_constant<int, 1>{});
    point_step(std::integral_constant<int, 0>{});
    const uint64_t half = L >> 1, at = j0 >> 1;
#pragma unroll
    for (int k = 0; k < 5; k++) {
        uint32_t* pe = out + (uint64_t)k * half + at;
        uint32_t* po = out + (uint64_t)(5 + k) * half + at;
        if constexpr (R == 4) {
            Fp e0 = ro[0].c[k], e1 = ro[2].c[k], o0 = ro[1].c[k], o1 = ro[3].c[k];
            if (accumulate) { const uint2 a = *reinterpret_cast<uint2*>(pe), b = *reinterpret_cast<uint2*>(po); e0 += Fp::raw(a.x); e1 += Fp::raw(a.y); o0 += Fp::raw(b.x); o1 += Fp::raw(b.y); }
            *reinterpret_cast<uint2*>(pe) = make_uint2(e0.v, e1.v);
            *reinterpret_cast<uint2*>(po) = make_uint2(o0.v, o1.v);
        } else {
            Fp e0 = ro[0].c[k], o0 = ro[1].c[k];
            if (accumulate) { e0 += Fp::raw(*pe); o0 += Fp::raw(*po); }
            *pe = e0.v;
            *po = o0.v;
        }
    }
}

__global__ void __launch_bounds__(256) k_fri_fold(const uint32_t* __restrict__ in, uint64_t L, const uint32_t* __restrict__ beta5 ,
                           const uint32_t* __restrict__ add, DeviceTables tb, uint32_t* __restrict__ out) {
    const uint64_t half = L >> 1;
// ... 193 lines not shown
```

### valida_amd/csrc/kernels/perm.hip

```cpp
#include <algorithm>
#include <cstdlib>
#include "launch.hpp"
#include "interactions.hpp"
#include "../chips/basic_machine.hpp"

namespace vk {

__global__ void __launch_bounds__(256) k_perm_recip(DMatView main, DMatView prep, const uint32_t* __restrict__ iw, const uint32_t* __restrict__ chal, DMatView perm) {
    uint64_t n = (uint64_t)blockIdx.x * blockDim.x + threadIdx.x;
    if (n >= main.height) return;
    const uint32_t M = iw[0];
    const uint32_t* betas = chal + 5 * M;
    Ext5 delta = Ext5::zero();
    for (uint32_t m = 0; m < M; m++) {
        uint32_t pos = iw[2 + m];
        const bool is_send = iw[pos] != 0;
        const uint32_t nf = iw[pos + 1];
        pos += 2;
        Fp mult = eval_vcol(iw, pos, main.data, main.stride, prep.data, prep.stride, n);
        Ext5 rlc = ext_from_words(chal + 5 * m);
        for (uint32_t j = 0; j < nf; j++) {
            Fp f = eval_vcol(iw, pos, main.data, main.stride, prep.data, prep.stride, n);
            rlc += ext_from_words(betas + 5 * j) * f;
        }
        Ext5 q = rlc.inv();
        store_ext(perm.data + (uint64_t)(5 * m) * perm.stride, perm.stride, n, q);
        Ext5 term = q * mult;
        delta = is_send ? delta + term : delta - term;
    }
    store_ext(perm.data + (uint64_t)(5 * M) * perm.stride, perm.stride, n, delta);
}

constexpr int PERM_NATIVE_MAX_M = 5;
struct DevicePermRow {
    const uint32_t* main;
    uint64_t stride;
    uint32_t roff;
    const uint32_t* chal;
    const uint32_t* betas;
    Ext5 rl[PERM_NATIVE_MAX_M];
    Fp mult[PERM_NATIVE_MAX_M];
    uint32_t snd;
    Ext5 rlc;
    uint64_t t[5];
    int pend, m, j;
    __device__ __forceinline__ Fp value(const vchips::Lin& f) const {
        Fp v = Fp::from_canonical(f.k);
#pragma unroll
        for (int i = 0; i < 4; i++)
            if (i < f.n) {
                const Fp x = Fp::raw(load_at(main + (uint64_t)f.col[i] * stride, roff));
                v += f.w[i] == 1u ? x : x * Fp::from_canonical(f.w[i]);
            }
        return v;
    }
    __device__ __forceinline__ void flush() {
#pragma unroll
        for (int c = 0; c < 5; c++) { rlc.c[c] += Fp::raw(vg::monty_reduce_wide(t[c])); t[c] = 0; }
        pend = 0;
    }
    __device__ __forceinline__ void begin(bool is_send, int) {
        snd |= (is_send ? 1u : 0u) << m;
        rlc = ext_from_words(chal + 5 * m);
#pragma unroll
        for (int c = 0; c < 5; c++) t[c] = 0;
        pend = 0; j = 0;
    }
    __device__ __forceinline__ void field(const vchips::Lin& f) {
        if (!(f.n == 0 && f.k == 0)) {
            const Fp x = value(f);
#pragma unroll
            for (int c = 0; c < 5; c++) t[c] += (uint64_t)betas[5 * j + c] * x.v;
            if (++pend == 4) flush();
        }
        j++;
    }
    __device__ __forceinline__ void end(const vchips::Lin& count) {
        if (pend) flush();
        const Fp cnt = value(count);
#pragma unroll
        for (int mm = 0; mm < PERM_NATIVE_MAX_M; mm++) if (mm == m) { rl[mm] = rlc; mult[mm] = cnt; }
        m++;
    }
};
template <int CHIP>
__device__ __forceinline__ Ext5 perm_row_native(const DMatView& main, const uint32_t* __restrict__ iw, const uint32_t* __restrict__ chal, const DMatView& perm, uint64_t n, int* m_out) {
    const uint32_t M = iw[0];
    DevicePermRow v;
    v.main = main.data; v.stride = main.stride; v.roff = (uint32_t)n * 4u;
    v.chal = chal; v.betas = chal + 5 * M;
    v.m = 0; v.pend = 0; v.j = 0; v.snd = 0;
    vchips::visit_interactions(CHIP, v);
    Ext5 pre[PERM_NATIVE_MAX_M];
    Ext5 run = Ext5::one();
#pragma unroll
    for (int m = 0; m < PERM_NATIVE_MAX_M; m++)
        if (m < v.m) { pre[m] = run; run = run * (v.rl[m].is_zero() ? Ext5::one() : v.rl[m]); }
    Ext5 inv = run.inv();
    Ext5 delta = Ext5::zero();
#pragma unroll
    for (int m = PERM_NATIVE_MAX_M - 1; m >= 0; m--)
        if (m < v.m) {
            const bool z = v.rl[m].is_zero();
            Ext5 q = inv * pre[m];
            inv = inv * (z ? Ext5::one() : v.rl[m]);
            if (z) q = Ext5::zero();
            store_ext(perm.data + (uint64_t)(5 * m) * perm.stride, perm.stride, n, q);
            const Ext5 term = q * v.mult[m];
            delta = ((v.snd >> m) & 1u) ? delta + term : delta - term;
        }
    *m_out = v.m;
    return delta;
}
template <int CHIP>
__global__ void __launch_bounds__(256) k_perm_recip_native(DMatView main, const uint32_t* __restrict__ iw, const uint32_t* __restrict__ chal, DMatView perm) {
    const uint64_t n = (uint64_t)blockIdx.x * blockDim.x + threadIdx.x;
    if (n >= main.height) return;
    int m;
    const Ext5 delta = perm_row_native<CHIP>(main, iw, chal, perm, n, &m);
    store_ext(perm.data + (uint64_t)(5 * m) * perm.stride, perm.stride, n, delta);
}


constexpr int SCAN_ITEMS = 4, SCAN_THREADS = 256, SCAN_BLOCK = SCAN_ITEMS * SCAN_THREADS;

#if defined(__HIPCC__) && !defined(HIPEMU_CHECKS)
__device__ __forceinline__ Fp block_exclusive_scan(Fp v, uint32_t* lds, Fp* total) {
    const int lane = (int)(threadIdx.x & 63), wave = (int)(threadIdx.x >> 6);
    Fp incl = v;
#pragma unroll
    for (int off = 1; off < 64; off <<= 1) {
        const Fp t = Fp::raw((uint32_t)__shfl_up((int)incl.v, off, 64));
        if (lane >= off) incl += t;
    }
    if (lane == 63) lds[wave] = incl.v;
    __syncthreads();
    Fp before = Fp::zero(), all = Fp::zero();
#pragma unroll
    for (int w = 0; w < SCAN_THREADS / 64; w++) {
        const Fp t = Fp::raw(lds[w]);
        all += t;
        if (w < wave) before += t;
    }
    __syncthreads();
    *total = all;
    return before + incl - v;
}
#else
__device__ __forceinline__ Fp block_exclusive_scan(Fp v, uint32_t* lds, Fp* total) {
    lds[threadIdx.x] = v.v;
    __syncthreads();
    for (int off = 1; off < SCAN_THREADS; off <<= 1) {
        Fp t = Fp::raw(lds[threadIdx.x]);
        if ((int)threadIdx.x >= off) t += Fp::raw(lds[threadIdx.x - off]);
        __syncthreads();
        lds[threadIdx.x] = t.v;
        __syncthreads();
    }
    *total = Fp::raw(lds[SCAN_THREADS - 1]);
    Fp incl = Fp::raw(lds[threadIdx.x]);
    __syncthreads();
    return incl - v;
}
#endif

static_assert(SCAN_ITEMS == 4, "scan_load4 / k_scan_apply move four consecutive elements as one uint4");
__device__ __forceinline__ void scan_load4(const uint32_t* col, uint64_t base, uint64_t n, bool vec, Fp (&v)[SCAN_ITEMS]) {
    if (vec && base + 4 <= n) {
        const uint4 q = *reinterpret_cast<const uint4*>(col + base);
        v[0] = Fp::raw(q.x); v[1] = Fp::raw(q.y); v[2] = Fp::raw(q.z); v[3] = Fp::raw(q.w);
        return;
    }
#pragma unroll
    for (int i = 0; i < SCAN_ITEMS; i++) v[i] = base + i < n ? Fp::raw(col[base + i]) : Fp::zero();
// ... 85 lines not shown
```

### valida_amd/csrc/kernels/quotient.hip

```cpp
#include <cstdlib>
#include <stdexcept>
#include "launch.hpp"
#include "interactions.hpp"
#include "../chips/basic_machine.hpp"

namespace vk {

struct PointCtx {
    uint64_t row, next_row;
    Fp is_first, is_last, is_trans;
};

typedef uint32_t v32u __attribute__((ext_vector_type(32)));

#define VG_INTERP_BODY(GET, SET)                                                                                                        \
    switch (in.op) {                                                                                                                    \
        case vair::OP_CONST: SET(in.dst, (uint32_t)in.a | ((uint32_t)in.b << 16)); break;                                               \
        case vair::OP_LOAD_MAIN: SET(in.dst, in.flag ? a.main_nx[(uint64_t)in.a * a.main_lde.stride + p.next_row] : a.main_lde.data[(uint64_t)in.a * a.main_lde.stride + p.row]); break; \
        case vair::OP_LOAD_PREP: SET(in.dst, in.flag ? a.prep_nx[(uint64_t)in.a * a.prep_lde.stride + p.next_row] : a.prep_lde.data[(uint64_t)in.a * a.prep_lde.stride + p.row]); break; \
        case vair::OP_SEL_FIRST: SET(in.dst, p.is_first.v); break;                                                                      \
        case vair::OP_SEL_LAST: SET(in.dst, p.is_last.v); break;                                                                        \
        case vair::OP_SEL_TRANS: SET(in.dst, p.is_trans.v); break;                                                                      \
        case vair::OP_ADD: { uint32_t x = GET(in.a), y = GET(in.b); SET(in.dst, (Fp::raw(x) + Fp::raw(y)).v); } break;                  \
        case vair::OP_SUB: { uint32_t x = GET(in.a), y = GET(in.b); SET(in.dst, (Fp::raw(x) - Fp::raw(y)).v); } break;                  \
        case vair::OP_MUL: { uint32_t x = GET(in.a), y = GET(in.b); SET(in.dst, (Fp::raw(x) * Fp::raw(y)).v); } break;                  \
        case vair::OP_NEG: { uint32_t x = GET(in.a); SET(in.dst, (-Fp::raw(x)).v); } break;                                             \
        case vair::OP_ASSERT: { uint32_t x = GET(in.a); acc += ext_from_words(a.consts + 5 * k) * Fp::raw(x); k++; } break;             \
        default: break;                                                                                             \
    }

template <int NB>
__device__ __forceinline__ Ext5 run_program_vgpr(const QuotientArgs& a, const PointCtx& p) {
    Ext5 acc = Ext5::zero();
    uint32_t k = 0;
    v32u r0 = {}, r1 = {};
#define VG_GET(i) (NB == 1 ? r0[(i) & 31] : ((i) < 32 ? r0[(i) & 31] : r1[(i) & 31]))
#define VG_SET(i, val) do { uint32_t _v = (val); if (NB == 1 || (i) < 32) r0[(i) & 31] = _v; else r1[(i) & 31] = _v; } while (0)
    for (uint32_t pc = 0; pc < a.n_instrs; pc += 4) {
        vair::Instr quad[4];
        __builtin_memcpy(quad, a.prog + pc, 32);
#pragma unroll
        for (int u = 0; u < 4; u++) {
            const vair::Instr in = quad[u];
            VG_INTERP_BODY(VG_GET, VG_SET)
        }
    }
#undef VG_GET
#undef VG_SET
    return acc;
}

__device__ __forceinline__ Ext5 run_program_lds(const QuotientArgs& a, const PointCtx& p, uint32_t* regs ) {
    Ext5 acc = Ext5::zero();
    uint32_t k = 0;
    const uint32_t S = blockDim.x;
    uint32_t* r = regs + threadIdx.x;
#define VG_GET(i) (r[(uint32_t)(i) * S])
#define VG_SET(i, val) (r[(uint32_t)(i) * S] = (val))
    for (uint32_t pc = 0; pc < a.n_instrs; pc++) {
        const vair::Instr in = a.prog[pc];
        VG_INTERP_BODY(VG_GET, VG_SET)
    }
#undef VG_GET
#undef VG_SET
    return acc;
}

#ifndef VGPU_QUOT_SADDR
#define VGPU_QUOT_SADDR 1
#endif
struct DeviceFolder {
    using Expr = Fp;
#if VGPU_QUOT_SADDR
    const uint32_t* __restrict__ main_p;
    const uint32_t* __restrict__ main_n;
    uint64_t mstride;
    const uint32_t* __restrict__ prep_p;
    const uint32_t* __restrict__ prep_n;
    uint64_t pstride;
    uint32_t roff, noff;
#else
    const uint32_t* __restrict__ main_p;
    const uint32_t* __restrict__ main_n;
    uint64_t mstride;
    const uint32_t* __restrict__ prep_p;
    const uint32_t* __restrict__ prep_n;
    uint64_t pstride;
#endif
    Fp first, last, trans;
    const uint32_t* __restrict__ apow;
    uint64_t t[5];
    Ext5 total;
    int k, pending;
    __device__ __forceinline__ Fp constant(uint32_t c) const { return Fp::from_canonical(c); }
#if VGPU_QUOT_SADDR
    __device__ __forceinline__ Fp main(int col, bool next) const { return Fp::raw(load_at((next ? main_n : main_p) + (uint64_t)col * mstride, next ? noff : roff)); }
    __device__ __forceinline__ Fp preprocessed(int col, bool next) const { return Fp::raw(load_at((next ? prep_n : prep_p) + (uint64_t)col * pstride, next ? noff : roff)); }
#else
    __device__ __forceinline__ Fp main(int col, bool next) const { return Fp::raw((next ? main_n : main_p)[(uint64_t)col * mstride]); }
    __device__ __forceinline__ Fp preprocessed(int col, bool next) const { return Fp::raw((next ? prep_n : prep_p)[(uint64_t)col * pstride]); }
#endif
    __device__ __forceinline__ Fp is_first_row() const { return first; }
    __device__ __forceinline__ Fp is_last_row() const { return last; }
    __device__ __forceinline__ Fp is_transition() const { return trans; }
    __device__ __forceinline__ void flush() {
#pragma unroll
        for (int c = 0; c < 5; c++) { total.c[c] += Fp::raw(vg::monty_reduce_wide(t[c])); t[c] = 0; }
        pending = 0;
    }
    __device__ __forceinline__ void assert_zero(const Fp& e) {
#pragma unroll
        for (int c = 0; c < 5; c++) t[c] += (uint64_t)apow[5 * k + c] * e.v;
        k++;
        if (++pending == 4) flush();
    }
};

template <int CHIP>
__device__ __forceinline__ Ext5 run_native(const QuotientArgs& a, const PointCtx& p) {
    if (CHIP < 0) return Ext5::zero();
    DeviceFolder f;
#if VGPU_QUOT_SADDR
    f.main_p = a.main_lde.data; f.main_n = a.main_nx; f.mstride = a.main_lde.stride;
    f.prep_p = a.prep_lde.data; f.prep_n = a.prep_nx; f.pstride = a.prep_lde.stride;
    f.roff = (uint32_t)p.row * 4u; f.noff = (uint32_t)p.next_row * 4u;
#else
    f.main_p = a.main_lde.data + p.row; f.main_n = a.main_nx + p.next_row; f.mstride = a.main_lde.stride;
    f.prep_p = a.prep_lde.data + p.row; f.prep_n = a.prep_nx + p.next_row; f.pstride = a.prep_lde.stride;
#endif
    f.first = p.is_first; f.last = p.is_last; f.trans = p.is_trans;
    f.apow = a.consts;
    f.total = Ext5::zero();
    f.k = 0; f.pending = 0;
#pragma unroll
    for (int c = 0; c < 5; c++) f.t[c] = 0;
    vchips::eval_chip(CHIP, f);
    if (f.pending) f.flush();
    return f.total;
}

__device__ __forceinline__ Ext5 load_ext_at(const uint32_t* ubase, uint64_t stride, uint32_t byte_off) {
    Ext5 e;
#pragma unroll
    for (int k = 0; k < 5; k++) e.c[k] = Fp::raw(load_at(ubase + (uint64_t)k * stride, byte_off));
    return e;
}
__device__ __forceinline__ Ext5 perm_constraints(const QuotientArgs& a, const PointCtx& p) {
    const uint32_t* iw = a.iw;
    const uint32_t M = iw[0], maxf = iw[1];
    const uint32_t* apow = a.consts + 5 * a.n_air_asserts;
    const uint32_t* bus = a.consts + 5 * a.K;
    const uint32_t* betas = bus + 5 * M;
    const Ext5 cumulative_sum = ext_from_words(betas + 5 * maxf);
    Ext5 acc = Ext5::zero(), rhs = Ext5::zero(), phi_0 = Ext5::zero();
    const uint32_t roff = (uint32_t)p.row * 4u, noff = (uint32_t)p.next_row * 4u;
    for (uint32_t m = 0; m < M; m++) {
        uint32_t pos = iw[2 + m];
        const bool is_send = iw[pos] != 0;
        const uint32_t nf = iw[pos + 1];
        pos += 2;
        uint32_t pos_n = pos;
        Fp mult_local = eval_vcol_at(iw, pos, a.main_lde.data, a.main_lde.stride, a.prep_lde.data, a.prep_lde.stride, roff);
        Fp mult_next = eval_vcol_at(iw, pos_n, a.main_nx, a.main_lde.stride, a.prep_nx, a.prep_lde.stride, noff);
        Ext5 rlc = ext_from_words(bus + 5 * m);
        for (uint32_t j0 = 0; j0 < nf; j0 += 4) {
            uint64_t t[5] = {0, 0, 0, 0, 0};
            const uint32_t je = nf - j0 < 4 ? nf - j0 : 4;
            for (uint32_t j = 0; j < je; j++) {
                Fp f = eval_vcol_at(iw, pos, a.main_lde.data, a.main_lde.stride, a.prep_lde.data, a.prep_lde.stride, roff);
#pragma unroll
                for (int c = 0; c < 5; c++) t[c] += (uint64_t)betas[5 * (j0 + j) + c] * f.v;
            }
#pragma unroll
            for (int c = 0; c < 5; c++) rlc.c[c] += Fp::raw(vg::monty_reduce_wide(t[c]));
        }
        const uint32_t* pcol = a.perm_lde.data + (uint64_t)(5 * m) * a.perm_lde.stride;
        Ext5 pl = load_ext_at(pcol, a.perm_lde.stride, roff), pn = load_ext_at(a.perm_nx + (uint64_t)(5 * m) * a.perm_lde.stride, a.perm_lde.stride, noff);
        acc += ext_from_words(apow + 5 * m) * (rlc * pl - Fp::one());
        Ext5 tl = pl * mult_local, tn = pn * mult_next;
        if (is_send) { phi_0 += tl; rhs += tn; } else { phi_0 -= tl; rhs -= tn; }
    }
    const uint32_t* phicol = a.perm_lde.data + (uint64_t)(5 * M) * a.perm_lde.stride;
    Ext5 phi_local = load_ext_at(phicol, a.perm_lde.stride, roff), phi_next = load_ext_at(a.perm_nx + (uint64_t)(5 * M) * a.perm_lde.stride, a.perm_lde.stride, noff);
    acc += ext_from_words(apow + 5 * M) * (((phi_next - phi_local) - rhs) * p.is_trans);
    acc += ext_from_words(apow + 5 * (M + 1)) * ((phi_local - phi_0) * p.is_first);
    acc += ext_from_words(apow + 5 * (M + 2)) * ((phi_local - cumulative_sum) * p.is_last);
    return acc;
}

struct DevicePerm {
    const QuotientArgs& a;
    uint32_t roff, noff;
    const uint32_t* apow;
    const uint32_t* bus;
    const uint32_t* betas;
    Ext5 acc, rhs, phi_0, rlc;
    uint64_t t[5];
    int pend, m, j;
    bool send;
    __device__ __forceinline__ Fp value(const vchips::Lin& f, bool next) const {
        Fp v = Fp::from_canonical(f.k);
#pragma unroll
        for (int i = 0; i < 4; i++)
            if (i < f.n) {
                const Fp x = Fp::raw(load_at((next ? a.main_nx : a.main_lde.data) + (uint64_t)f.col[i] * a.main_lde.stride, next ? noff : roff));
                v += f.w[i] == 1u ? x : x * Fp::from_canonical(f.w[i]);
            }
        return v;
    }
    __device__ __forceinline__ void flush() {
#pragma unroll
        for (int c = 0; c < 5; c++) { rlc.c[c] += Fp::raw(vg::monty_reduce_wide(t[c])); t[c] = 0; }
        pend = 0;
    }
    __device__ __forceinline__ void begin(bool is_send, int) {
        send = is_send;
        rlc = ext_from_words(bus + 5 * m);
#pragma unroll
        for (int c = 0; c < 5; c++) t[c] = 0;
        pend = 0; j = 0;
    }
    __device__ __forceinline__ void field(const vchips::Lin& f) {
        if (!(f.n == 0 && f.k == 0)) {
            const Fp x = value(f, false);
#pragma unroll
            for (int c = 0; c < 5; c++) t[c] += (uint64_t)betas[5 * j + c] * x.v;
            if (++pend == 4) flush();
        }
        j++;
    }
    __device__ __forceinline__ void end(const vchips::Lin& count) {
        if (pend) flush();
        const Fp mult_local = value(count, false), mult_next = value(count, true);
        const Ext5 pl = load_ext_at(a.perm_lde.data + (uint64_t)(5 * m) * a.perm_lde.stride, a.perm_lde.stride, roff);
        const Ext5 pn = load_ext_at(a.perm_nx + (uint64_t)(5 * m) * a.perm_lde.stride, a.perm_lde.stride, noff);
        acc += ext_from_words(apow + 5 * m) * (rlc * pl - Fp::one());
        const Ext5 tl = pl * mult_local, tn = pn * mult_next;
        if (send) { phi_0 += tl; rhs += tn; } else { phi_0 -= tl; rhs -= tn; }
        m++;
    }
};
template <int CHIP>
__device__ __forceinline__ Ext5 perm_constraints_native(const QuotientArgs& a, const PointCtx& p) {
    const uint32_t M = a.iw[0], maxf = a.iw[1];
    DevicePerm v{a, (uint32_t)p.row * 4u, (uint32_t)p.next_row * 4u, a.consts + 5 * a.n_air_asserts, a.consts + 5 * a.K, a.consts + 5 * a.K + 5 * M,
                 Ext5::zero(), Ext5::zero(), Ext5::zero(), Ext5::zero(), {0, 0, 0, 0, 0}, 0, 0, 0, false};
    vchips::visit_interactions(CHIP, v);
    const Ext5 cumulative_sum = ext_from_words(v.betas + 5 * maxf);
    const Ext5 phi_local = load_ext_at(a.perm_lde.data + (uint64_t)(5 * v.m) * a.perm_lde.stride, a.perm_lde.stride, v.roff);
    const Ext5 phi_next = load_ext_at(a.perm_nx + (uint64_t)(5 * v.m) * a.perm_lde.stride, a.perm_lde.stride, v.noff);
    Ext5 acc = v.acc;
    acc += ext_from_words(v.apow + 5 * v.m) * (((phi_next - phi_local) - v.rhs) * p.is_trans);
    acc += ext_from_words(v.apow + 5 * (v.m + 1)) * ((phi_local - v.phi_0) * p.is_first);
    acc += ext_from_words(v.apow + 5 * (v.m + 2)) * ((phi_local - cumulative_sum) * p.is_last);
    return acc;
}

template <int RFKIND, int CHIP = -1>
__global__ void __launch_bounds__(256) k_quotient(QuotientArgs a, DeviceTables tb) {
    extern __shared__ uint32_t regs[];
    const uint64_t n = 1ull << a.log_n;
    uint64_t m = (uint64_t)blockIdx.x * blockDim.x + threadIdx.x;
#ifndef VGPU_QUOT_TILE
#define VGPU_QUOT_TILE 1
#endif
    const bool tiled = VGPU_QUOT_TILE && a.log_n >= 9 && blockDim.x == 256;
    const bool nat_tile = tiled && a.out_natural;
    if (nat_tile) {
        m = ((uint64_t)(threadIdx.x >> 4) << (a.log_n - 4)) | ((uint64_t)blockIdx.x << 4) | (threadIdx.x & 15u);
    } else if (tiled) {
        const uint32_t B = blockIdx.x, top = B >> (a.log_n - 9), mid = B & ((1u << (a.log_n - 9)) - 1u);
        m = ((uint64_t)top << (a.log_n - 1)) | ((uint64_t)(threadIdx.x >> 5) << (a.log_n - 4)) | ((uint64_t)mid << 5) | (threadIdx.x & 31u);
    }
    if (m >= n) return;
    const int kq = a.log_n + 1;
    const uint32_t Qmask = (uint32_t)(2 * n - 1);
    const uint32_t j0 = (uint32_t)(2 * m), j1 = j0 + 1;
    const uint32_t i0 = vg::reverse_bits_len((uint32_t)m, (unsigned)a.log_n);
    const uint32_t i1 = i0 + (uint32_t)n;
    const Fp s = Fp::raw(a.coset_shift), g_inv = Fp::raw(a.g_inv);
    const Fp x0 = s * domain_point(tb, j0), x1 = -x0;
    Fp d00 = x0 - Fp::one(), d01 = x0 - g_inv, d10 = x1 - Fp::one(), d11 = x1 - g_inv;
    Fp p01 = d00 * d01, p23 = d10 * d11;
    Fp inv_all = (p01 * p23).inv();
    Fp ip01 = inv_all * p23, ip23 = inv_all * p01;
    Fp id00 = ip01 * d01, id01 = ip01 * d00, id10 = ip23 * d11, id11 = ip23 * d10;
    const uint32_t par0 = i0 & 1u, par1 = i1 & 1u;
    PointCtx p0, p1;
    p0.row = j0; p0.next_row = vg::reverse_bits_len((i0 + a.next_step_p1 - 1u) & Qmask, (unsigned)kq);
    p1.row = j1; p1.next_row = vg::reverse_bits_len((i1 + a.next_step_p1 - 1u) & Qmask, (unsigned)kq);
    p0.is_trans = d01; p0.is_first = Fp::raw(a.zh[par0]) * id00; p0.is_last = Fp::raw(a.zh[par0]) * id01;
    p1.is_trans = d11; p1.is_first = Fp::raw(a.zh[par1]) * id10; p1.is_last = Fp::raw(a.zh[par1]) * id11;
    Ext5 q0 = Ext5::zero(), q1 = Ext5::zero();
#pragma unroll 1
    for (int pt = 0; pt < 2; pt++) {
        PointCtx p;
        p.row = pt ? p1.row : p0.row; p.next_row = pt ? p1.next_row : p0.next_row;
        p.is_first = pt ? p1.is_first : p0.is_first; p.is_last = pt ? p1.is_last : p0.is_last; p.is_trans = pt ? p1.is_trans : p0.is_trans;
        Ext5 q;
        if (RFKIND == 3) q = run_native<CHIP>(a, p);
        else if (RFKIND == 0) q = run_program_lds(a, p, regs);
        else q = run_program_vgpr<RFKIND>(a, p);
        q = (q + perm_constraints(a, p)) * Fp::raw(a.zh_inv[pt ? par1 : par0]);
        if (pt) q1 = q; else q0 = q;
    }
    Fp x0_inv = Fp::raw(a.coset_shift_inv) * inv_domain_point(tb, j0);
    Ext5 sum = q0 + q1, diff = (q0 - q1) * x0_inv;
    if (nat_tile) {
        __shared__ uint32_t tr[10 * 256];
        const uint32_t A = threadIdx.x >> 4, r = threadIdx.x & 15u, slot = (r << 4) | (__brev(A) >> 28);
#pragma unroll
        for (int c = 0; c < 5; c++) { tr[c * 256 + slot] = sum.c[c].halve().v; tr[(5 + c) * 256 + slot] = diff.c[c].halve().v; }
        __syncthreads();
        const uint64_t row = ((uint64_t)(__brev(A) >> 28) << (a.log_n - 4)) | ((uint64_t)(a.log_n > 8 ? __brev((uint32_t)blockIdx.x) >> (32 - (a.log_n - 8)) : 0u) << 4) | r;
#pragma unroll
        for (int c = 0; c < 10; c++) a.out.data[(uint64_t)c * a.out.stride + row] = tr[c * 256 + threadIdx.x];
        return;
    }
    const uint64_t pos = a.out_natural ? (uint64_t)i0 : m;
#pragma unroll
    for (int c = 0; c < 5; c++) {
        a.out.data[(uint64_t)c * a.out.stride + pos] = sum.c[c].halve().v;
        a.out.data[(uint64_t)(5 + c) * a.out.stride + pos] = diff.c[c].halve().v;
    }
}

#ifndef VGPU_QUOT_PT_WAVES
#define VGPU_QUOT_PT_WAVES 6
#endif
// ... 253 lines not shown
```

Before: 68.06 proofs/s.

## Use lazy Montgomery accumulation with folded high word across field dot products

Introduces a LazyAcc/ExtAcc accumulator that sums 64-bit products and folds the high word (a single conditional subtract) instead of doing a full Montgomery reduction every four terms, so each dot product needs only one final reduction. It is applied to Ext5 multiplication, opening reductions, permutation RLC accumulation and quotient constraint folding, with single-sum variants for most chips. A probe kernel and API are added to test correctness. The risk is extra fold branches and register pressure from the five 64-bit accumulators with room counters, plus subtle overflow-bound reasoning.

```diff
diff --git a/bindings/rust/src/lib.rs b/bindings/rust/src/lib.rs
--- a/bindings/rust/src/lib.rs
+++ b/bindings/rust/src/lib.rs
@@ -382,6 +382,7 @@
     pub fn vgpu_host_commit_root(cfg: *const VgpuConfig, mats: *const *const u32, heights: *const u64, widths: *const u64, n_mats: u32, coset_shifts: *const u32, root: *mut u32) -> i32;
     pub fn vgpu_fri_fold(p: *mut VgpuProver, f: *const u32, n: u64, beta: *const u32, out: *mut u32) -> i32;
     pub fn vgpu_field_probe(p: *mut VgpuProver, op: u32, operands: *const u32, operand_words: u64, n_items: u64, results: *mut u32, result_words: u64) -> i32;
+    pub fn vgpu_lazy_probe(p: *mut VgpuProver, op: u32, terms: u32, operands: *const u32, operand_words: u64, n_items: u64, results: *mut u32, result_words: u64) -> i32;
     pub fn vgpu_prover_set_pool_poison(p: *mut VgpuProver, mode: u32, word: u32) -> i32;
     pub fn vgpu_prover_pool_poison_stats(p: *const VgpuProver, out: *mut u64);
     pub fn vgpu_prover_pool_peek(p: *mut VgpuProver, bytes: u64, out: *mut u32, n_words: u64) -> i32;
diff --git a/include/vgpu.h b/include/vgpu.h
--- a/include/vgpu.h
+++ b/include/vgpu.h
@@ -160,6 +160,8 @@
 int32_t vgpu_fri_fold(vgpu_prover_t* p, const uint32_t* f, uint64_t n, const uint32_t beta[5], uint32_t* out);
 
 int32_t vgpu_field_probe(vgpu_prover_t* p, uint32_t op, const uint32_t* operands, uint64_t operand_words, uint64_t n_items, uint32_t* results, uint64_t result_words);
+
+int32_t vgpu_lazy_probe(vgpu_prover_t* p, uint32_t op, uint32_t terms, const uint32_t* operands, uint64_t operand_words, uint64_t n_items, uint32_t* results, uint64_t result_words);
 
 int32_t vgpu_prover_set_pool_poison(vgpu_prover_t* p, uint32_t mode, uint32_t word);
 void vgpu_prover_pool_poison_stats(const vgpu_prover_t* p, uint64_t out[4]);
diff --git a/valida_amd/__init__.py b/valida_amd/__init__.py
--- a/valida_amd/__init__.py
+++ b/valida_amd/__init__.py
@@ -347,6 +347,27 @@
     out = np.zeros((ow, n), dtype=np.uint32)
     _check(lib().vgpu_field_probe(prover._h, ctypes.c_uint32(code), src.ctypes.data_as(c_u32p), ctypes.c_uint64(src.size), ctypes.c_uint64(n),
                                   out.ctypes.data_as(c_u32p), ctypes.c_uint64(out.size)))
+    return np.ascontiguousarray(out.T)
+
+
+LAZY_PROBE_OPS = {name: (code, iw, ow, tuple(terms)) for code, (name, iw, ow, terms) in enumerate([
+    ("fold_hi", lambda n: 2, 2, (0,)), ("ext_mul", lambda n: 10, 5, (0,)), ("lin_dot", lambda n: 6 * n, 5, list(range(1, 18)) + [34]),
+    ("ext_dot", lambda n: 10 * n, 5, range(1, 9)), ("lin_dot_loop", lambda n: 6 * n, 5, range(1, 65))])}
+
+
+def lazy_probe(prover, op, terms, operands):
+    code, iwf, ow, lengths = LAZY_PROBE_OPS[op]
+    if terms not in lengths:
+        raise ValueError("lazy_probe(%s): no such length %r" % (op, terms))
+    iw = iwf(terms)
+    a = np.ascontiguousarray(operands, dtype=np.uint32)
+    if a.ndim != 2 or a.shape[1] != iw or a.shape[0] == 0:
+        raise ValueError("lazy_probe(%s, %d): operands must be a non-empty (n_items, %d) array" % (op, terms, iw))
+    n = a.shape[0]
+    src = np.ascontiguousarray(a.T)
+    out = np.zeros((ow, n), dtype=np.uint32)
+    _check(lib().vgpu_lazy_probe(prover._h, ctypes.c_uint32(code), ctypes.c_uint32(terms), src.ctypes.data_as(c_u32p), ctypes.c_uint64(src.size), ctypes.c_uint64(n),
+                                 out.ctypes.data_as(c_u32p), ctypes.c_uint64(out.size)))
     return np.ascontiguousarray(out.T)
 
 
diff --git a/valida_amd/build.py b/valida_amd/build.py
--- a/valida_amd/build.py
+++ b/valida_amd/build.py
@@ -34,6 +34,7 @@
     "kernels/memory_audit.hip",
     "kernels/program_audit.hip",
     "kernels/field_probe.hip",
+    "kernels/lazy_probe.hip",
     "host/prover.cpp",
     "host/prover_audits.cpp",
     "host/sharded_prover.cpp",
diff --git a/valida_amd/csrc/capi.cpp b/valida_amd/csrc/capi.cpp
--- a/valida_amd/csrc/capi.cpp
+++ b/valida_amd/csrc/capi.cpp
@@ -911,6 +911,23 @@
     })
 }
 
+int32_t vgpu_lazy_probe(vgpu_prover_t* p, uint32_t op, uint32_t terms, const uint32_t* operands, uint64_t operand_words, uint64_t n_items, uint32_t* results, uint64_t result_words) {
+    VG_TRY({
+        int iw = 0, ow = 0;
+        if (!p || !operands || !results) throw std::invalid_argument("null argument");
+        if (!vk::lazy_probe_shape(op, terms, &iw, &ow)) throw std::invalid_argument("lazy probe: unknown op or length");
+        if (n_items == 0 || n_items > (1ull << 24)) throw std::invalid_argument("lazy probe: 1 .. 2^24 items");
+        if (operand_words != n_items * (uint64_t)iw || result_words != n_items * (uint64_t)ow) throw std::invalid_argument("lazy probe: buffer sizes do not match the op's shape");
+        DeviceCtx& c = p->p->ctx();
+        c.activate();
+        DBuf din(&c, (size_t)operand_words), dout(&c, (size_t)result_words);
+        c.upload(din.data, operands, operand_words * 4);
+        vk::launch_lazy_probe(c.stream, op, terms, din.data, n_items, dout.data);
+        c.check_launch("lazy probe");
+        c.download(results, dout.data, result_words * 4);
+    })
+}
+
 int32_t vgpu_prover_set_pool_poison(vgpu_prover_t* p, uint32_t mode, uint32_t word) {
     VG_TRY({
         if (!p) throw std::invalid_argument("null argument");
diff --git a/valida_amd/csrc/field.hpp b/valida_amd/csrc/field.hpp
--- a/valida_amd/csrc/field.hpp
+++ b/valida_amd/csrc/field.hpp
@@ -94,6 +94,59 @@
     uint32_t u = mul_hi_u32(m, P);
     return sub_mod(hi, u);
 }
+
+VG_HD uint64_t fold_hi(uint64_t t) { return ((uint64_t)reduce_once((uint32_t)(t >> 32)) << 32) | (uint32_t)t; }
+
+#ifndef VG_LAZY_CHECK
+#define VG_LAZY_CHECK 0
+#endif
+#if VG_LAZY_CHECK
+[[noreturn]] void lazy_check_failed(const char* what, uint64_t t);
+#endif
+struct LazyAcc {
+    uint64_t t;
+    int room;
+#if VG_LAZY_CHECK
+    unsigned __int128 shadow;
+    inline void check_hi(const char* what) const {
+        if (shadow != (unsigned __int128)t) lazy_check_failed("the 64-bit sum wrapped", t);
+        if ((uint32_t)(t >> 32) >= 2u * P) lazy_check_failed(what, t);
+    }
+#endif
+    VG_HD void clear() {
+        t = 0; room = 4;
+#if VG_LAZY_CHECK
+        shadow = 0;
+#endif
+    }
+    VG_HD static LazyAcc zero() { LazyAcc a; a.clear(); return a; }
+    VG_HD void fold() {
+#if VG_LAZY_CHECK
+        check_hi("high word >= 2p at a fold");
+#endif
+        t = fold_hi(t); room = 2;
+#if VG_LAZY_CHECK
+        shadow = t;
+#endif
+    }
+    template <int W> VG_HD void add_product(uint32_t a, uint32_t b) {
+        if (room < W) fold();
+        room -= W;
+#if VG_LAZY_CHECK
+        shadow += (unsigned __int128)((uint64_t)a * b);
+        if (shadow >> 64) lazy_check_failed("the 64-bit sum would wrap", t);
+#endif
+        t += (uint64_t)a * b;
+    }
+    VG_HD void mac(uint32_t a, uint32_t b) { add_product<1>(a, b); }
+    VG_HD void mac2(uint32_t a, uint32_t b) { add_product<2>(a, b); }
+    VG_HD uint32_t reduce() const {
+#if VG_LAZY_CHECK
+        check_hi("high word >= 2p at the final reduction");
+#endif
+        return monty_reduce_wide(t);
+    }
+};
 
 struct Fp {
     uint32_t v;
@@ -165,12 +218,10 @@
         Ext5 r;
 #pragma unroll
         for (int k = 0; k < 5; k++) {
-            uint32_t bb[5];
-#pragma unroll
-            for (int i = 0; i < 5; i++) bb[i] = i <= k ? o.c[k - i].v : d[k + 5 - i].v;
-            uint64_t t0123 = (uint64_t)c[0].v * bb[0] + (uint64_t)c[1].v * bb[1] + (uint64_t)c[2].v * bb[2] + (uint64_t)c[3].v * bb[3];
-            uint64_t t4 = (uint64_t)c[4].v * bb[4];
-            r.c[k] = Fp::raw(monty_reduce_wide(t0123)) + Fp::raw(monty_reduce(t4));
+            LazyAcc acc = LazyAcc::zero();
+#pragma unroll
+            for (int i = 0; i < 5; i++) acc.mac(c[i].v, i <= k ? o.c[k - i].v : d[k + 5 - i].v);
+            r.c[k] = Fp::raw(acc.reduce());
         }
         return r;
     }
@@ -204,6 +255,29 @@
     }
 };
 
+struct ExtAcc {
+    LazyAcc l[5];
+    VG_HD static ExtAcc zero() { ExtAcc a; for (int k = 0; k < 5; k++) a.l[k].clear(); return a; }
+    VG_HD void mac(const uint32_t* a5, uint32_t v) {
+#pragma unroll
+        for (int k = 0; k < 5; k++) l[k].mac(a5[k], v);
+    }
+    VG_HD void mac(const Ext5& a, const Fp& v) {
+#pragma unroll
+        for (int k = 0; k < 5; k++) l[k].mac(a.c[k].v, v.v);
+    }
+    VG_HD void mac(const Ext5& a, const Ext5& b) {
+        Fp d[5];
+#pragma unroll
+        for (int j = 0; j < 5; j++) d[j] = b.c[j] + b.c[j];
+#pragma unroll
+        for (int k = 0; k < 5; k++)
+#pragma unroll
+            for (int i = 0; i < 5; i++) l[k].mac(a.c[i].v, i <= k ? b.c[k - i].v : d[k + 5 - i].v);
+    }
+    VG_HD Ext5 reduce() const { Ext5 r; for (int k = 0; k < 5; k++) r.c[k] = Fp::raw(l[k].reduce()); return r; }
+};
+
 VG_HD uint32_t reverse_bits_len(uint32_t x, unsigned bits) {
 #if defined(__HIP_DEVICE_COMPILE__)
     return bits ? (__brev(x) >> (32 - bits)) : 0;
diff --git a/valida_amd/csrc/kernels/launch.hpp b/valida_amd/csrc/kernels/launch.hpp
--- a/valida_amd/csrc/kernels/launch.hpp
+++ b/valida_amd/csrc/kernels/launch.hpp
@@ -63,6 +63,9 @@
 bool field_probe_shape(uint32_t op, int* in_words, int* out_words);
 void field_probe_check_twiddle_range(uint32_t op, const uint32_t* in_host, uint64_t n);
 void launch_field_probe(hipStream_t st, uint32_t op, const uint32_t* in_dev, uint64_t n, const DeviceTables& tb, const uint32_t* pos_dev, bool sparse, uint32_t* out_dev);
+enum LazyProbeOp { LP_FOLD_HI = 0, LP_EXT_MUL, LP_LIN_DOT, LP_EXT_DOT, LP_LIN_DOT_LOOP, LAZY_PROBE_OPS };
+bool lazy_probe_shape(uint32_t op, uint32_t terms, int* in_words, int* out_words);
+void launch_lazy_probe(hipStream_t st, uint32_t op, uint32_t terms, const uint32_t* in_dev, uint64_t n, uint32_t* out_dev);
 void launch_intt(hipStream_t st, DMatView m, const DeviceTables& tb);
 void launch_coset_ntt(hipStream_t st, DMatView coeffs, DMatView dst, uint64_t dst_row0, Fp shift, const DeviceTables& tb);
 void launch_lde_natural(hipStream_t st, DMatView nat, DMatView lde, int log_blowup, const DeviceTables& tb, const LdeTables& lt, DMatView s1, DMatView s2,
diff --git a/valida_amd/csrc/kernels/lazy_probe.hip b/valida_amd/csrc/kernels/lazy_probe.hip
--- /dev/null
+++ b/valida_amd/csrc/kernels/lazy_probe.hip
@@ -0,0 +1,76 @@
+#include "launch.hpp"
+#include <stdexcept>
+
+namespace vk {
+
+bool lazy_probe_shape(uint32_t op, uint32_t terms, int* in_words, int* out_words) {
+    switch (op) {
+        case LP_FOLD_HI: if (terms != 0) return false; *in_words = 2; *out_words = 2; return true;
+        case LP_EXT_MUL: if (terms != 0) return false; *in_words = 10; *out_words = 5; return true;
+        case LP_LIN_DOT: if (!((terms >= 1 && terms <= 17) || terms == 34)) return false; *in_words = 6 * (int)terms; *out_words = 5; return true;
+        case LP_EXT_DOT: if (terms < 1 || terms > 8) return false; *in_words = 10 * (int)terms; *out_words = 5; return true;
+        case LP_LIN_DOT_LOOP: if (terms < 1 || terms > 64) return false; *in_words = 6 * (int)terms; *out_words = 5; return true;
+        default: return false;
+    }
+}
+
+template <int OP, int N>
+__global__ void __launch_bounds__(256) k_lazy_probe(const uint32_t* __restrict__ in, uint64_t n, uint32_t terms, uint32_t* __restrict__ out) {
+    const uint64_t i = (uint64_t)blockIdx.x * blockDim.x + threadIdx.x;
+    if (i >= n) return;
+    auto a = [&](int k) { return in[(uint64_t)k * n + i]; };
+    auto put = [&](int k, uint32_t v) { out[(uint64_t)k * n + i] = v; };
+    auto ext = [&](int k0) { Ext5 e; for (int k = 0; k < 5; k++) e.c[k] = Fp::raw(a(k0 + k)); return e; };
+    auto put_e = [&](const Ext5& e) { for (int k = 0; k < 5; k++) put(k, e.c[k].v); };
+    if constexpr (OP == LP_FOLD_HI) {
+        const uint64_t t = vg::fold_hi(((uint64_t)a(1) << 32) | a(0));
+        put(0, (uint32_t)t);
+        put(1, (uint32_t)(t >> 32));
+    } else if constexpr (OP == LP_EXT_MUL) {
+        put_e(ext(0) * ext(5));
+    } else if constexpr (OP == LP_LIN_DOT) {
+        vg::ExtAcc acc = vg::ExtAcc::zero();
+#pragma unroll
+        for (int c = 0; c < N; c++) acc.mac(ext(6 * c), Fp::raw(a(6 * c + 5)));
+        put_e(acc.reduce());
+    } else if constexpr (OP == LP_EXT_DOT) {
+        vg::ExtAcc acc = vg::ExtAcc::zero();
+#pragma unroll
+        for (int c = 0; c < N; c++) acc.mac(ext(10 * c), ext(10 * c + 5));
+        put_e(acc.reduce());
+    } else {
+        vg::ExtAcc acc = vg::ExtAcc::zero();
+#pragma unroll 1
+        for (uint32_t c = 0; c < terms; c++) acc.mac(ext(6 * (int)c), Fp::raw(a(6 * (int)c + 5)));
+        put_e(acc.reduce());
+    }
+}
+
+template <int OP, int N, int NMAX>
+static void lazy_probe_terms(hipStream_t st, uint32_t terms, const uint32_t* in, uint64_t n, uint32_t* out) {
+    if constexpr (N <= NMAX) {
+        if (terms == (uint32_t)N) { VK_LAUNCH((k_lazy_probe<OP, N>), dim3((unsigned)((n + 255) / 256)), dim3(256), 0, st, in, n, terms, out); return; }
+        lazy_probe_terms<OP, N + 1, NMAX>(st, terms, in, n, out);
+    }
+}
+
+void launch_lazy_probe(hipStream_t st, uint32_t op, uint32_t terms, const uint32_t* in_dev, uint64_t n, uint32_t* out_dev) {
+    int iw, ow;
+    if (!lazy_probe_shape(op, terms, &iw, &ow)) throw std::invalid_argument("lazy probe: unknown op or length");
+    if (!n) return;
+    if (n > (1ull << 24)) throw std::invalid_argument("lazy probe: at most 2^24 items per launch");
+    ProfScope ps("k_lazy_probe", st, 0.0);
+    const dim3 grid((unsigned)((n + 255) / 256)), block(256);
+    switch (op) {
+        case LP_FOLD_HI: VK_LAUNCH((k_lazy_probe<LP_FOLD_HI, 0>), grid, block, 0, st, in_dev, n, terms, out_dev); break;
+        case LP_EXT_MUL: VK_LAUNCH((k_lazy_probe<LP_EXT_MUL, 0>), grid, block, 0, st, in_dev, n, terms, out_dev); break;
+        case LP_LIN_DOT:
+            if (terms == 34) VK_LAUNCH((k_lazy_probe<LP_LIN_DOT, 34>), grid, block, 0, st, in_dev, n, terms, out_dev);
+            else lazy_probe_terms<LP_LIN_DOT, 1, 17>(st, terms, in_dev, n, out_dev);
+            break;
+        case LP_EXT_DOT: lazy_probe_terms<LP_EXT_DOT, 1, 8>(st, terms, in_dev, n, out_dev); break;
+        default: VK_LAUNCH((k_lazy_probe<LP_LIN_DOT_LOOP, 0>), grid, block, 0, st, in_dev, n, terms, out_dev); break;
+    }
+}
+
+}
diff --git a/valida_amd/csrc/kernels/open.hip b/valida_amd/csrc/kernels/open.hip
--- a/valida_amd/csrc/kernels/open.hip
+++ b/valida_amd/csrc/kernels/open.hip
@@ -300,33 +300,23 @@
         const uint64_t stride = ((uint64_t)md[3] << 32) | md[2];
         const uint32_t width = md[4], npts = md[5];
         md += 6;
-        Ext5 rr = Ext5::zero();
+        vg::ExtAcc ra = vg::ExtAcc::zero();
         uint32_t c = 0;
         for (; c + 16 <= width; c += 16) {
             uint32_t v[16];
 #pragma unroll
             for (int u = 0; u < 16; u++) v[u] = colp[(uint64_t)(c + u) * stride + j];
 #pragma unroll
-            for (int g = 0; g < 16; g += 4) {
-                const uint32_t* a0 = apow + 5 * (c + g);
-#pragma unroll
-                for (int k = 0; k < 5; k++) {
-                    uint64_t t = (uint64_t)a0[k] * v[g] + (uint64_t)a0[5 + k] * v[g + 1] + (uint64_t)a0[10 + k] * v[g + 2] + (uint64_t)a0[15 + k] * v[g + 3];
-                    rr.c[k] += Fp::raw(vg::monty_reduce_wide(t));
-                }
-            }
+            for (int u = 0; u < 16; u++) ra.mac(apow + 5 * (c + u), v[u]);
         }
         for (; c + 4 <= width; c += 4) {
             const uint32_t v0 = colp[(uint64_t)c * stride + j], v1 = colp[(uint64_t)(c + 1) * stride + j];
             const uint32_t v2 = colp[(uint64_t)(c + 2) * stride + j], v3 = colp[(uint64_t)(c + 3) * stride + j];
             const uint32_t* a0 = apow + 5 * c;
-#pragma unroll
-            for (int k = 0; k < 5; k++) {
-                uint64_t t = (uint64_t)a0[k] * v0 + (uint64_t)a0[5 + k] * v1 + (uint64_t)a0[10 + k] * v2 + (uint64_t)a0[15 + k] * v3;
-                rr.c[k] += Fp::raw(vg::monty_reduce_wide(t));
-            }
-        }
-        for (; c < width; c++) rr += ext_from_words(apow + 5 * c) * Fp::raw(colp[(uint64_t)c * stride + j]);
+            ra.mac(a0, v0); ra.mac(a0 + 5, v1); ra.mac(a0 + 10, v2); ra.mac(a0 + 15, v3);
+        }
+        for (; c < width; c++) ra.mac(apow + 5 * c, colp[(uint64_t)c * stride + j]);
+        const Ext5 rr = ra.reduce();
         for (uint32_t q = 0; q < npts; q++, md += 11) {
             Ext5 t = ext_from_words(md + 1) * (ext_from_words(md + 6) - rr);
             const uint32_t slot = md[0];
@@ -387,41 +377,50 @@
         const uint64_t stride = ((uint64_t)md[3] << 32) | md[2];
         const uint32_t width = md[4], npts = md[5];
         md += 6;
+        vg::ExtAcc ra[R];
+#pragma unroll
+        for (int r = 0; r < R; r++) ra[r] = vg::ExtAcc::zero();
+        auto one_col = [&](const V& v, const uint32_t* a0) {
+            uint32_t e[R];
+            RowVec<R>::get(v, e);
+#pragma unroll
+            for (int r = 0; r < R; r++) ra[r].mac(a0, e[r]);
+        };
+        auto eight_cols = [&](uint32_t c0) {
+            V v[8];
+#pragma unroll
+            for (int u = 0; u < 8; u++) v[u] = *reinterpret_cast<const V*>(colp + (uint64_t)(c0 + u) * stride);
+#pragma unroll
+            for (int u = 0; u < 8; u++) one_col(v[u], apow + 5 * (c0 + u));
+        };
+        auto last_col = [&](uint32_t c0) { one_col(*reinterpret_cast<const V*>(colp + (uint64_t)c0 * stride), apow + 5 * c0); };
+        uint32_t c = 0;
+        if (width >= 8) {
+            eight_cols(0);
+            for (c = 8; c + 8 <= width; c += 8) eight_cols(c);
+        }
+#pragma unroll
+        for (int r = 0; r < R; r++)
+#pragma unroll
+            for (int k = 0; k < 5; k++) ra[r].l[k].room = 0;
+        if (c + 4 <= width) {
+            V v[4];
+#pragma unroll
+            for (int u = 0; u < 4; u++) v[u] = *reinterpret_cast<const V*>(colp + (uint64_t)(c + u) * stride);
+#pragma unroll
+            for (int u = 0; u < 4; u++) one_col(v[u], apow + 5 * (c + u));
+            c += 4;
+        }
+        if (c < width) {
+            last_col(c);
+            if (c + 1 < width) {
+                last_col(c + 1);
+                if (c + 2 < width) last_col(c + 2);
+            }
+        }
         Ext5 rr[R];
 #pragma unroll
-        for (int r = 0; r < R; r++) rr[r] = Ext5::zero();
-        auto four_cols = [&](const V& v0, const V& v1, const V& v2, const V& v3, const uint32_t* a0) {
-            uint32_t e0[R], e1[R], e2[R], e3[R];
-            RowVec<R>::get(v0, e0); RowVec<R>::get(v1, e1); RowVec<R>::get(v2, e2); RowVec<R>::get(v3, e3);
-#pragma unroll
-            for (int r = 0; r < R; r++)
-#pragma unroll
-                for (int k = 0; k < 5; k++) {
-                    const uint64_t t = (uint64_t)a0[k] * e0[r] + (uint64_t)a0[5 + k] * e1[r] + (uint64_t)a0[10 + k] * e2[r] + (uint64_t)a0[15 + k] * e3[r];
-                    rr[r].c[k] += Fp::raw(vg::monty_reduce_wide(t));
-                }
-        };
-        uint32_t c = 0;
-        for (; c + 8 <= width; c += 8) {
-            V v[8];
-#pragma unroll
-            for (int u = 0; u < 8; u++) v[u] = *reinterpret_cast<const V*>(colp + (uint64_t)(c + u) * stride);
-            four_cols(v[0], v[1], v[2], v[3], apow + 5 * c);
-            four_cols(v[4], v[5], v[6], v[7], apow + 5 * (c + 4));
-        }
-        for (; c + 4 <= width; c += 4) {
-            V v[4];
-#pragma unroll
-            for (int u = 0; u < 4; u++) v[u] = *reinterpret_cast<const V*>(colp + (uint64_t)(c + u) * stride);
-            four_cols(v[0], v[1], v[2], v[3], apow + 5 * c);
-        }
-        for (; c < width; c++) {
-            uint32_t e[R];
-            RowVec<R>::get(*reinterpret_cast<const V*>(colp + (uint64_t)c * stride), e);
-            const Ext5 a = ext_from_words(apow + 5 * c);
-#pragma unroll
-            for (int r = 0; r < R; r++) rr[r] += a * Fp::raw(e[r]);
-        }
+        for (int r = 0; r < R; r++) rr[r] = ra[r].reduce();
         for (uint32_t q = 0; q < npts; q++, md += 11) {
             const Ext5 coef = ext_from_words(md + 1), Y = ext_from_words(md + 6);
             const uint32_t slot = md[0];
diff --git a/valida_amd/csrc/kernels/perm.hip b/valida_amd/csrc/kernels/perm.hip
--- a/valida_amd/csrc/kernels/perm.hip
+++ b/valida_amd/csrc/kernels/perm.hip
@@ -18,11 +18,12 @@
         const uint32_t nf = iw[pos + 1];
         pos += 2;
         Fp mult = eval_vcol(iw, pos, main.data, main.stride, prep.data, prep.stride, n);
-        Ext5 rlc = ext_from_words(chal + 5 * m);
+        vg::ExtAcc t = vg::ExtAcc::zero();
         for (uint32_t j = 0; j < nf; j++) {
             Fp f = eval_vcol(iw, pos, main.data, main.stride, prep.data, prep.stride, n);
-            rlc += ext_from_words(betas + 5 * j) * f;
-        }
+            t.mac(betas + 5 * j, f.v);
+        }
+        const Ext5 rlc = ext_from_words(chal + 5 * m) + t.reduce();
         Ext5 q = rlc.inv();
         store_ext(perm.data + (uint64_t)(5 * m) * perm.stride, perm.stride, n, q);
         Ext5 term = q * mult;
@@ -41,9 +42,8 @@
     Ext5 rl[PERM_NATIVE_MAX_M];
     Fp mult[PERM_NATIVE_MAX_M];
     uint32_t snd;
-    Ext5 rlc;
-    uint64_t t[5];
-    int pend, m, j;
+    vg::ExtAcc t;
+    int m, j;
     __device__ __forceinline__ Fp value(const vchips::Lin& f) const {
         Fp v = Fp::from_canonical(f.k);
 #pragma unroll
@@ -54,29 +54,20 @@
             }
         return v;
     }
-    __device__ __forceinline__ void flush() {
-#pragma unroll
-        for (int c = 0; c < 5; c++) { rlc.c[c] += Fp::raw(vg::monty_reduce_wide(t[c])); t[c] = 0; }
-        pend = 0;
-    }
     __device__ __forceinline__ void begin(bool is_send, int) {
         snd |= (is_send ? 1u : 0u) << m;
-        rlc = ext_from_words(chal + 5 * m);
-#pragma unroll
-        for (int c = 0; c < 5; c++) t[c] = 0;
-        pend = 0; j = 0;
+        t = vg::ExtAcc::zero();
+        j = 0;
     }
     __device__ __forceinline__ void field(const vchips::Lin& f) {
         if (!(f.n == 0 && f.k == 0)) {
             const Fp x = value(f);
-#pragma unroll
-            for (int c = 0; c < 5; c++) t[c] += (uint64_t)betas[5 * j + c] * x.v;
-            if (++pend == 4) flush();
+            t.mac(betas + 5 * j, x.v);
         }
         j++;
     }
     __device__ __forceinline__ void end(const vchips::Lin& count) {
-        if (pend) flush();
+        const Ext5 rlc = ext_from_words(chal + 5 * m) + t.reduce();
         const Fp cnt = value(count);
 #pragma unroll
         for (int mm = 0; mm < PERM_NATIVE_MAX_M; mm++) if (mm == m) { rl[mm] = rlc; mult[mm] = cnt; }
@@ -89,7 +80,7 @@
     DevicePermRow v;
     v.main = main.data; v.stride = main.stride; v.roff = (uint32_t)n * 4u;
     v.chal = chal; v.betas = chal + 5 * M;
-    v.m = 0; v.pend = 0; v.j = 0; v.snd = 0;
+    v.m = 0; v.j = 0; v.snd = 0; v.t = vg::ExtAcc::zero();
     vchips::visit_interactions(CHIP, v);
     Ext5 pre[PERM_NATIVE_MAX_M];
     Ext5 run = Ext5::one();
diff --git a/valida_amd/csrc/kernels/quotient.hip b/valida_amd/csrc/kernels/quotient.hip
--- a/valida_amd/csrc/kernels/quotient.hip
+++ b/valida_amd/csrc/kernels/quotient.hip
@@ -69,6 +69,7 @@
 #ifndef VGPU_QUOT_SADDR
 #define VGPU_QUOT_SADDR 1
 #endif
+template <bool ONE_SUM>
 struct DeviceFolder {
     using Expr = Fp;
 #if VGPU_QUOT_SADDR
@@ -89,9 +90,9 @@
 #endif
     Fp first, last, trans;
     const uint32_t* __restrict__ apow;
-    uint64_t t[5];
+    vg::ExtAcc t;
     Ext5 total;
-    int k, pending;
+    int k;
     __device__ __forceinline__ Fp constant(uint32_t c) const { return Fp::from_canonical(c); }
 #if VGPU_QUOT_SADDR
     __device__ __forceinline__ Fp main(int col, bool next) const { return Fp::raw(load_at((next ? main_n : main_p) + (uint64_t)col * mstride, next ? noff : roff)); }
@@ -103,23 +104,21 @@
     __device__ __forceinline__ Fp is_first_row() const { return first; }
     __device__ __forceinline__ Fp is_last_row() const { return last; }
     __device__ __forceinline__ Fp is_transition() const { return trans; }
-    __device__ __forceinline__ void flush() {
-#pragma unroll
-        for (int c = 0; c < 5; c++) { total.c[c] += Fp::raw(vg::monty_reduce_wide(t[c])); t[c] = 0; }
-        pending = 0;
-    }
     __device__ __forceinline__ void assert_zero(const Fp& e) {
-#pragma unroll
-        for (int c = 0; c < 5; c++) t[c] += (uint64_t)apow[5 * k + c] * e.v;
+        t.mac(apow + 5 * k, e.v);
         k++;
-        if (++pending == 4) flush();
+        if (!ONE_SUM && t.l[0].room == 0) { total += t.reduce(); t = vg::ExtAcc::zero(); }
+    }
+    __device__ __forceinline__ Ext5 sum() const {
+        if (ONE_SUM) return t.reduce();
+        return t.l[0].room != 4 ? total + t.reduce() : total;
     }
 };
 
 template <int CHIP>
 __device__ __forceinline__ Ext5 run_native(const QuotientArgs& a, const PointCtx& p) {
     if (CHIP < 0) return Ext5::zero();
-    DeviceFolder f;
+    DeviceFolder<CHIP != vchips::CHIP_CPU> f;
 #if VGPU_QUOT_SADDR
     f.main_p = a.main_lde.data; f.main_n = a.main_nx; f.mstride = a.main_lde.stride;
     f.prep_p = a.prep_lde.data; f.prep_n = a.prep_nx; f.pstride = a.prep_lde.stride;
@@ -130,13 +129,11 @@
 #endif
     f.first = p.is_first; f.last = p.is_last; f.trans = p.is_trans;
     f.apow = a.consts;
+    f.t = vg::ExtAcc::zero();
     f.total = Ext5::zero();
-    f.k = 0; f.pending = 0;
-#pragma unroll
-    for (int c = 0; c < 5; c++) f.t[c] = 0;
+    f.k = 0;
     vchips::eval_chip(CHIP, f);
-    if (f.pending) f.flush();
-    return f.total;
+    return f.sum();
 }
 
 __device__ __forceinline__ Ext5 load_ext_at(const uint32_t* ubase, uint64_t stride, uint32_t byte_off) {
@@ -162,18 +159,12 @@
         uint32_t pos_n = pos;
         Fp mult_local = eval_vcol_at(iw, pos, a.main_lde.data, a.main_lde.stride, a.prep_lde.data, a.prep_lde.stride, roff);
         Fp mult_next = eval_vcol_at(iw, pos_n, a.main_nx, a.main_lde.stride, a.prep_nx, a.prep_lde.stride, noff);
-        Ext5 rlc = ext_from_words(bus + 5 * m);
-        for (uint32_t j0 = 0; j0 < nf; j0 += 4) {
-            uint64_t t[5] = {0, 0, 0, 0, 0};
-            const uint32_t je = nf - j0 < 4 ? nf - j0 : 4;
-            for (uint32_t j = 0; j < je; j++) {
-                Fp f = eval_vcol_at(iw, pos, a.main_lde.data, a.main_lde.stride, a.prep_lde.data, a.prep_lde.stride, roff);
-#pragma unroll
-                for (int c = 0; c < 5; c++) t[c] += (uint64_t)betas[5 * (j0 + j) + c] * f.v;
-            }
-#pragma unroll
-            for (int c = 0; c < 5; c++) rlc.c[c] += Fp::raw(vg::monty_reduce_wide(t[c]));
-        }
+        vg::ExtAcc t = vg::ExtAcc::zero();
+        for (uint32_t j = 0; j < nf; j++) {
+            Fp f = eval_vcol_at(iw, pos, a.main_lde.data, a.main_lde.stride, a.prep_lde.data, a.prep_lde.stride, roff);
+            t.mac(betas + 5 * j, f.v);
+        }
+        const Ext5 rlc = ext_from_words(bus + 5 * m) + t.reduce();
         const uint32_t* pcol = a.perm_lde.data + (uint64_t)(5 * m) * a.perm_lde.stride;
         Ext5 pl = load_ext_at(pcol, a.perm_lde.stride, roff), pn = load_ext_at(a.perm_nx + (uint64_t)(5 * m) * a.perm_lde.stride, a.perm_lde.stride, noff);
         acc += ext_from_words(apow + 5 * m) * (rlc * pl - Fp::one());
@@ -188,6 +179,7 @@
     return acc;
 }
 
+template <bool ONE_SUM>
 struct DevicePerm {
     const QuotientArgs& a;
     uint32_t roff, noff;
@@ -195,8 +187,8 @@
     const uint32_t* bus;
     const uint32_t* betas;
     Ext5 acc, rhs, phi_0, rlc;
-    uint64_t t[5];
-    int pend, m, j;
+    vg::ExtAcc t;
+    int m, j;
     bool send;
     __device__ __forceinline__ Fp value(const vchips::Lin& f, bool next) const {
         Fp v = Fp::from_canonical(f.k);
@@ -208,29 +200,22 @@
             }
         return v;
     }
-    __device__ __forceinline__ void flush() {
-#pragma unroll
-        for (int c = 0; c < 5; c++) { rlc.c[c] += Fp::raw(vg::monty_reduce_wide(t[c])); t[c] = 0; }
-        pend = 0;
-    }
     __device__ __forceinline__ void begin(bool is_send, int) {
         send = is_send;
         rlc = ext_from_words(bus + 5 * m);
-#pragma unroll
-        for (int c = 0; c < 5; c++) t[c] = 0;
-        pend = 0; j = 0;
+        t = vg::ExtAcc::zero();
+        j = 0;
     }
     __device__ __forceinline__ void field(const vchips::Lin& f) {
         if (!(f.n == 0 && f.k == 0)) {
             const Fp x = value(f, false);
-#pragma unroll
-            for (int c = 0; c < 5; c++) t[c] += (uint64_t)betas[5 * j + c] * x.v;
-            if (++pend == 4) flush();
+            t.mac(betas + 5 * j, x.v);
+            if (!ONE_SUM && t.l[0].room == 0) { rlc += t.reduce(); t = vg::ExtAcc::zero(); }
         }
         j++;
     }
     __device__ __forceinline__ void end(const vchips::Lin& count) {
-        if (pend) flush();
+        if (ONE_SUM || t.l[0].room != 4) rlc += t.reduce();
         const Fp mult_local = value(count, false), mult_next = value(count, true);
         const Ext5 pl = load_ext_at(a.perm_lde.data + (uint64_t)(5 * m) * a.perm_lde.stride, a.perm_lde.stride, roff);
         const Ext5 pn = load_ext_at(a.perm_nx + (uint64_t)(5 * m) * a.perm_lde.stride, a.perm_lde.stride, noff);
@@ -243,8 +228,8 @@
 template <int CHIP>
 __device__ __forceinline__ Ext5 perm_constraints_native(const QuotientArgs& a, const PointCtx& p) {
     const uint32_t M = a.iw[0], maxf = a.iw[1];
-    DevicePerm v{a, (uint32_t)p.row * 4u, (uint32_t)p.next_row * 4u, a.consts + 5 * a.n_air_asserts, a.consts + 5 * a.K, a.consts + 5 * a.K + 5 * M,
-                 Ext5::zero(), Ext5::zero(), Ext5::zero(), Ext5::zero(), {0, 0, 0, 0, 0}, 0, 0, 0, false};
+    DevicePerm<CHIP != vchips::CHIP_SHIFT> v{a, (uint32_t)p.row * 4u, (uint32_t)p.next_row * 4u, a.consts + 5 * a.n_air_asserts, a.consts + 5 * a.K, a.consts + 5 * a.K + 5 * M,
+                 Ext5::zero(), Ext5::zero(), Ext5::zero(), Ext5::zero(), vg::ExtAcc::zero(), 0, 0, false};
     vchips::visit_interactions(CHIP, v);
     const Ext5 cumulative_sum = ext_from_words(v.betas + 5 * maxf);
     const Ext5 phi_local = load_ext_at(a.perm_lde.data + (uint64_t)(5 * v.m) * a.perm_lde.stride, a.perm_lde.stride, v.roff);
```

New measurement: 69.45 proofs/s (median of 6 runs). +2.0%, better.
